# tangtang888/video-edge-ai-proxy

Measured on AMD Instinct MI355X. Metric: decoded FPS (whole node) + p50 VideoLatestImage latency, 256×1080p RTSP, higher is better.
Workload: dtype uint8 (BGR24 frames; bf16-capable consumer path)

## Files before the change

### csrc/bindings.cpp

```cpp
#include <malloc.h>

#include <pybind11/numpy.h>
#include <pybind11/pybind11.h>
#include <pybind11/stl.h>

#include "vep/hostprof.h"
#include "vep/avc.h"
#include "vep/avc_cavlc.h"
#include "vep/avc_recon.h"
#include "vep/bench_driver.h"
#include "vep/cabac.h"
#include "vep/codec.h"
#include "vep/gpu.h"
#include "vep/h264.h"
#include "vep/hevc_ctu.h"
#include "vep/hevc_dec.h"
#include "vep/hevc_kern.h"
#include "vep/jpeg.h"
#include "vep/scale.h"
#include "bind_ext.h"
#include "vep/runtime.h"
#include "vep/synth.h"

namespace py = pybind11;
// ... 837 lines not shown
  });
  m.def("parse_hevc_sps", [](const std::string& nal) {
    std::vector<u8> r(nal.size());
    size_t n = ebsp_to_rbsp(reinterpret_cast<const u8*>(nal.data()), nal.size(), r.data());
    hevc::Sps s = hevc::parse_sps(r.data(), n);
    py::dict d;
    d["profile_idc"] = s.ptl.profile_idc;
    d["level_idc"] = s.ptl.level_idc;
    d["width"] = s.out_width();
    d["height"] = s.out_height();
    d["coded_width"] = s.width;
    d["coded_height"] = s.height;
    d["fps"] = s.fps();
    d["ctb_size"] = s.ctb_size();
    d["pcm"] = s.pcm;
    d["num_short_term_rps"] = int(s.st_rps.size());
    d["scaling_list"] = s.scaling_list;
    d["scaling_list_data"] = s.scaling_list_data;
    d["long_term_refs"] = s.long_term_refs;
    d["num_long_term_ref_pics_sps"] = s.num_long_term_ref_pics_sps;
    return d;
  });
  auto hevc_rbsp = [](const std::string& nal) {
    std::vector<u8> r(nal.size());
    r.resize(ebsp_to_rbsp(reinterpret_cast<const u8*>(nal.data()), nal.size(), r.data()));
    return r;
  };
  m.def("parse_hevc_pps", [hevc_rbsp](const std::string& nal) {
    const std::vector<u8> r = hevc_rbsp(nal);
    hevc::Pps p = hevc::parse_pps(r.data(), r.size());
    py::dict d;
    d["tiles"] = p.tiles;
    d["tile_cols"] = p.tile_cols;
    d["tile_rows"] = p.tile_rows;
    d["uniform_spacing"] = p.uniform_spacing;
    d["loop_filter_across_tiles"] = p.loop_filter_across_tiles;
    d["entropy_coding_sync"] = p.entropy_coding_sync;
    d["dependent_slice_segments"] = p.dependent_slice_segments;
    d["weighted_pred"] = p.weighted_pred;
    d["weighted_bipred"] = p.weighted_bipred;
    d["transquant_bypass"] = p.transquant_bypass;
    d["scaling_list"] = p.scaling_list;
    return d;
  });
  m.def("hevc_scaling_factors", [hevc_rbsp](int size_id, int matrix_id, py::object sps_nal, py::object pps_nal) {
    VEP_CHECK(size_id >= 0 && size_id < 4 && matrix_id >= 0 && matrix_id < 6, "bad sizeId / matrixId");
    hevc::ScalingList sl;
    if (!sps_nal.is_none()) {
      const std::vector<u8> r = hevc_rbsp(sps_nal.cast<std::string>());
      sl = hevc::parse_sps(r.data(), r.size()).sl;
    }
    if (!pps_nal.is_none()) {
      const std::vector<u8> r = hevc_rbsp(pps_nal.cast<std::string>());
      hevc::Pps p = hevc::parse_pps(r.data(), r.size());
      if (p.scaling_list) sl = p.sl;
    }
    const int n = 4 << size_id;
    std::vector<u8> f(size_t(n) * n);
    sl.factors(size_id, matrix_id, f.data());
    return std::vector<int>(f.begin(), f.end());
  }, py::arg("size_id"), py::arg("matrix_id"), py::arg("sps_nal") = py::none(), py::arg("pps_nal") = py::none());
  m.def("hevc_slice_entry_points", [hevc_rbsp](const std::string& nal, const std::string& sps_nal,
                                               const std::string& pps_nal) {
    const std::vector<u8> rs = hevc_rbsp(sps_nal), rp = hevc_rbsp(pps_nal), r = hevc_rbsp(nal);
    const hevc::Sps sps = hevc::parse_sps(rs.data(), rs.size());
    const hevc::Pps pps = hevc::parse_pps(rp.data(), rp.size());
    const hevc::SliceHeader prev;
    const hevc::SliceHeader sh = hevc::parse_slice_header(r.data(), r.size(), sps, pps, &prev);
    size_t ebsp = 0, rbsp = 0;
    int zeros = 0;
    const u8* p = reinterpret_cast<const u8*>(nal.data());
    while (rbsp < sh.data_bytepos && ebsp < nal.size()) {
      const u8 b = p[ebsp++];
      if (zeros >= 2 && b == 3) {
        zeros = 0;
        continue;
      }
      ++rbsp;
      zeros = b == 0 ? zeros + 1 : 0;
    }
    py::dict d;
    d["entry_points"] = std::vector<u32>(sh.entry_points.begin(), sh.entry_points.end());
    d["data_offset_ebsp"] = ebsp;
    d["dependent"] = sh.dependent;
    d["segment_address"] = sh.segment_address;
    return d;
  });
  m.def("sparse_coef_fuzz", [](u64 seed, int trials) {
    u64 x = seed * 0x9E3779B97F4A7C15ull + 1;
    auto rnd = [&]() {
      x ^= x << 13;
      x ^= x >> 7;
      x ^= x << 17;
      return x;
    };
    auto val = [&](int density) -> i16 {
      if (int(rnd() & 15) >= density) return 0;
      const int r = int(rnd() % 8);
      if (r == 0) return i16(-32768);
      if (r == 1) return i16(32767);
      const int v = int(rnd() % 64) - 32;
      return i16(v ? v : 1);
    };
    int bad_avc = 0, bad_hevc = 0;
    for (int t = 0; t < trials; ++t) {
      const int dens = int(rnd() % 17);
      avc::MbResidual res;
      res.t8 = rnd() & 1;
      i16 want[avc::kDenseCoefs] = {};
      if (res.t8) {
        for (int q = 0; q < 4; ++q) {
          const bool coded = rnd() & 1;
          for (int i = 0; i < 64; ++i) want[64 * q + i] = res.b8[q][i] = coded ? val(dens) : 0;
          if (coded) res.luma |= u16(0x33u << ((q & 1) * 2 + (q >> 1) * 8));
        }
      } else {
        for (int b = 0; b < 16; ++b) {
          const bool coded = rnd() & 1;
          for (int i = 0; i < 16; ++i) want[16 * b + i] = res.blk[b][i] = coded ? val(dens) : 0;
          if (coded) res.luma |= u16(1u << b);
        }
      }
      for (int k = 0; k < 8; ++k) {
        const bool coded = rnd() & 1;
        for (int i = 0; i < 16; ++i) want[256 + 16 * k + i] = res.blk[16 + k][i] = coded ? val(dens) : 0;
        if (coded) res.chroma |= u8(1u << k);
      }
      avc::Picture pic;
      pic.wmbs = pic.hmbs = 1;
      pic.mbs.resize(1);
      avc::MbRec rec{};
      rec.kind = res.t8 ? avc::kI8x8 : avc::kI16x16;
      rec.flags = res.t8 ? u8(avc::kMbT8x8) : u8(0);
      avc::MbState s;
      avc::store_mb(pic, 0, rec, s, &res, nullptr);
      i16 got[avc::kDenseCoefs];
      avc::expand_coefs(pic.coefs.data(), pic.mbs[0], got);
      bad_avc += std::memcmp(got, want, sizeof got) != 0 ||
                 pic.coefs.size() != size_t(avc::coef_words(pic.mbs[0])) + avc::coef_values(pic.coefs.data(), pic.mbs[0]);
      for (int log2 = 2; log2 <= 5; ++log2) {
        const int nn = 1 << (2 * log2);
        std::vector<i16> dense(size_t(nn), 0), val_list, out(size_t(nn + nn / 16)), back(static_cast<size_t>(nn));
        std::vector<u16> pos;
        for (int k = 0; k < nn; ++k)
          if ((dense[size_t(k)] = val(dens))) pos.push_back(u16(k));
        for (size_t i = pos.size(); i > 1; --i) std::swap(pos[i - 1], pos[size_t(rnd() % i)]);
        for (u16 k : pos) val_list.push_back(dense[k]);
        const int n = hevc::hk_sparse_store(log2, pos.data(), val_list.data(), int(pos.size()), out.data());
        hevc::hk_sparse_expand(out.data(), log2, back.data());
        bad_hevc += back != dense || n != hevc::hk_sparse_words(log2) + int(pos.size());
      }
    }
    return std::make_pair(bad_avc, bad_hevc);
  });
  m.def("avc_parse_seconds", [](const std::vector<std::shared_ptr<AccessUnit>>& aus, int reps) {
    py::gil_scoped_release r;
    double best = 1e30;
    for (int k = 0; k < std::max(1, reps); ++k) {
      avc::Decoder dec;
      const i64 t0 = mono_us();
      for (const auto& au : aus) {
        size_t nal = 0;
        do dec.parse(*au, 0, &nal);
        while (nal < au->nals.size());
      }
      best = std::min(best, double(mono_us() - t0) * 1e-6);
    }
    return best;
  }, py::arg("aus"), py::arg("reps") = 3);
  m.def("avc_record_stats", [](const std::vector<std::shared_ptr<AccessUnit>>& aus) {
    py::gil_scoped_release r;
    avc::Decoder dec;
    u64 mbs = 0, coefs = 0, nz = 0, mvs = 0, pics = 0;
    for (const auto& au : aus) {
      auto p = dec.parse(*au);
      if (!p) continue;
      ++pics;
      mbs += p->mbs.size();
      coefs += p->coefs.size();
      mvs += p->mvs.size();
      for (const avc::MbRec& m : p->mbs)
        if (m.kind != avc::kIPcm) nz += avc::coef_values(p->coefs.data(), m);
    }
    py::gil_scoped_acquire g;
    py::dict d;
    d["pictures"] = pics;
    d["mbs"] = mbs;
    d["coefs"] = coefs;
    d["nonzero"] = nz;
    d["mvs"] = mvs;
    return d;
  });
  m.def("hevc_record_stats", [](const std::vector<std::shared_ptr<AccessUnit>>& aus) {
    py::gil_scoped_release r;
    hevc::Decoder dec;
    dec.set_gpu_mode(true);
    u64 pics = 0, tus = 0, coefs = 0, nz = 0, pus = 0;
    for (const auto& au : aus) {
      dec.decode(*au);
      for (const auto& p : dec.take_gpu_pictures()) {
        ++pics;
        tus += p->tus.size();
        pus += p->pus.size();
        coefs += p->coefs.size();
        for (i16 c : p->coefs) nz += c != 0;
      }
    }
    py::gil_scoped_acquire g;
    py::dict d;
    d["pictures"] = pics;
    d["tus"] = tus;
    d["coefs"] = coefs;
    d["nonzero"] = nz;
    d["pus"] = pus;
    return d;
  });
  m.def("avc_intra8x8_tap_check", [](u64 seed, int trials) {
    u64 st = seed * 0x9E3779B97F4A7C15ull + 7;
    auto rnd = [&]() {
      st ^= st << 13;
      st ^= st >> 7;
      st ^= st << 17;
      return int(st & 255);
    };
    int bad = 0;
    for (int t = 0; t < trials; ++t) {
      int s[25];
      for (int k = 0; k < 25; ++k) s[k] = (t & 3) == 0 ? (rnd() & 1) * 255 : rnd();
      auto T = [&](int i) { return s[1 + i]; };
      auto L = [&](int j) { return j < 0 ? s[0] : s[17 + j]; };
      for (int mode = 0; mode < 9; ++mode) {
        if (mode == 2) continue;
        for (int y = 0; y < 8; ++y)
          for (int x = 0; x < 8; ++x) {
            const u32 tw = avc::intra8x8_pred_tap(mode, x, y);
            const int got = avc::eval_tap8(tw, s[tw & 31], s[(tw >> 5) & 31], s[(tw >> 10) & 31]);
            bad += got != avc::intra8x8_pred_g(T, L, true, true, mode, x, y);
          }
      }
      for (int av = 0; av < 8; ++av) {
        const bool top = av & 1, left = av & 2, tl = av & 4;
        for (int k = 0; k < 25; ++k) {
          const u32 tw = avc::intra8x8_filter_tap(top, left, tl, k);
          const int got =
              (tw & avc::kTap8Const) ? 128 : avc::eval_tap8(tw, s[tw & 31], s[(tw >> 5) & 31], s[(tw >> 10) & 31]);
          bad += got != avc::intra8x8_filter_at(T, [&](int j) { return s[17 + j]; }, top, left, tl, k);
        }
      }
    }
    return bad;
  });
  m.def("cabac_roundtrip", [](u64 seed, int n, int qp) {
    u64 st = seed * 0x9E3779B97F4A7C15ull + 1;
    auto rnd = [&]() { st ^= st << 13; st ^= st >> 7; st ^= st << 17; return st; };
    const size_t nn = static_cast<size_t>(n);
    std::vector<u8> kind(nn), ctx(nn), bin(nn);
    for (int i = 0; i < n; ++i) {
      u64 r = rnd();
      kind[size_t(i)] = u8((r & 15) == 0 ? 1 : ((r & 63) == 1 ? 2 : 0));
      ctx[size_t(i)] = u8((r >> 8) % 4);
      const int p = ctx[size_t(i)] == 0 ? 2 : ctx[size_t(i)] == 1 ? 50 : ctx[size_t(i)] == 2 ? 97 : ((i / 500) & 1) ? 90 : 10;
      bin[size_t(i)] = kind[size_t(i)] == 2 ? 0 : u8(int((r >> 20) % 100) < p);
    }
    std::vector<u8> buf;
    cabac::Ctx ce[4], cd[4];
    const int init[4] = {197, 154, 122, 139};
    for (int k = 0; k < 4; ++k) ce[k].init(init[k], qp), cd[k].init(init[k], qp);
    {
      cabac::Encoder e(buf);
      for (int i = 0; i < n; ++i) {
        if (kind[size_t(i)] == 0) e.decision(ce[ctx[size_t(i)]], bin[size_t(i)]);
        else if (kind[size_t(i)] == 1) e.bypass(bin[size_t(i)]);
        else e.terminate(0);
      }
      e.terminate(1);
      e.align_zero();
    }
    cabac::Decoder d(buf.data(), buf.size(), 0);
    bool ok = true;
    for (int i = 0; i < n && ok; ++i) {
      u32 b;
      if (kind[size_t(i)] == 0) b = d.decision(cd[ctx[size_t(i)]]);
      else if (kind[size_t(i)] == 1) b = d.bypass();
      else b = d.terminate();
      ok = b == bin[size_t(i)];
    }
    ok = ok && d.terminate() == 1 && d.aligned_bytepos() == buf.size();
    return py::make_tuple(ok, buf.size());
  });
  m.def("parse_cost_us", [](const AccessUnit& au, int iters, std::shared_ptr<AccessUnit> prime) {
    py::gil_scoped_release r;
    StreamParser p;
    MbUpdate u;
    if (prime) p.absorb_parameter_sets(*prime);
    p.parse(au, u);
    i64 t0 = mono_us();
    for (int k = 0; k < iters; ++k) {
      u.clear_payload();
      p.parse(au, u);
    }
    const double parse_us = double(mono_us() - t0) / iters;
    std::vector<u32> epb;
    t0 = mono_us();
    for (int k = 0; k < iters; ++k)
      for (size_t i = 0; i < au.nals.size(); ++i) find_epb(au.nal(i), au.nal_size(i), epb);
    const double scan_us = double(mono_us() - t0) / iters;
// ... 1223 lines not shown
```

### csrc/vep/avc.cpp

```cpp
#include "avc.h"

#include <immintrin.h>

#include <algorithm>
#include <array>

#include "avc_cavlc.h"
#include "avc_internal.h"
#include "fanout.h"

namespace vep::avc {

using h264::Pps;
using h264::Sps;


void MbNeighbours::reset(int wmbs, int hmbs, bool ring) {
  w_ = wmbs;
  h_ = hmbs;
  cur_ = -1;
  run_slice_ = ~0u;
  run_start_ = 0;
  announced_ = 0;
  const size_t n = size_t(wmbs) * hmbs;
  if (++epoch_ == 0) {
    epoch_ = 1;
    stamp_.clear();
  }
  size_t ns = n;
  mask_ = ~size_t(0);
  if (ring) {
    size_t r = 1;
    while (r < 2 * (size_t(wmbs) + 2)) r <<= 1;
    if (r < n) {
      ns = r;
      mask_ = r - 1;
    }
  }
  if (st_.size() != ns) st_.assign(ns, MbState{});
  if (tag_.size() != ns) tag_.assign(ns, ~0u);
  if (stamp_.size() != n) stamp_.assign(n, 0u);
}

static int coded_count(const MbState& s, int blk) {
  if (s.kind == kSkip) return 0;
  if (s.kind == kIPcm) return 16;
  return s.tc[blk];
}

int MbNeighbours::nc_luma(int mb, int blk) const {
  const int bx = blk & 3, by = blk >> 2;
  int na = -1, nb = -1;
  const int am = mb_at(mb, bx * 4 - 1, by * 4);
  if (am >= 0) na = coded_count(st_[size_t(am) & mask_], bx > 0 ? blk - 1 : blk + 3);
  const int bm = mb_at(mb, bx * 4, by * 4 - 1);
  if (bm >= 0) nb = coded_count(st_[size_t(bm) & mask_], by > 0 ? blk - 4 : blk + 12);
  if (na >= 0 && nb >= 0) return (na + nb + 1) >> 1;
  if (na >= 0) return na;
  if (nb >= 0) return nb;
  return 0;
}

int MbNeighbours::nc_chroma(int mb, int c, int blk, int nbc) const {
  const int bx = blk & 1, by = blk >> 1;
  auto count = [&](int m, int b) {
    const MbState& s = st_[size_t(m) & mask_];
    if (s.kind == kSkip) return 0;
    if (s.kind == kIPcm) return 16;
    return int(s.tcc[c][b]);
  };
  int na = -1, nb = -1;
  const int am = bx > 0 ? mb : mb_at(mb, -1, 0);
  if (am >= 0) na = count(am, bx > 0 ? blk - 1 : blk + 1);
  const int bm = by > 0 ? mb : mb_at(mb, 0, -1);
  if (bm >= 0) nb = count(bm, by > 0 ? blk - 2 : blk + nbc - 2);
  if (na >= 0 && nb >= 0) return (na + nb + 1) >> 1;
  if (na >= 0) return na;
  if (nb >= 0) return nb;
  return 0;
}

int MbNeighbours::pred_intra4x4(int mb, int blk, bool constrained) const {
  const int bx = blk & 3, by = blk >> 2;
  const int am = mb_at(mb, bx * 4 - 1, by * 4), bm = mb_at(mb, bx * 4, by * 4 - 1);
  if (am < 0 || bm < 0) return 2;
  const MbState& a = st_[size_t(am) & mask_];
  const MbState& b = st_[size_t(bm) & mask_];
  if (constrained && (!is_intra(a.kind) || !is_intra(b.kind))) return 2;
  const int ma = a.kind == kI4x4 ? a.i4[bx > 0 ? blk - 1 : blk + 3] : 2;
  const int mbm = b.kind == kI4x4 ? b.i4[by > 0 ? blk - 4 : blk + 12] : 2;
  return ma < mbm ? ma : mbm;
}

int MbNeighbours::pred_intra8x8(int mb, int b8, bool constrained) const {
  const int blk = (b8 & 1) * 2 + (b8 >> 1) * 8;
  const int bx = blk & 3, by = blk >> 2;
  const int am = mb_at(mb, bx * 4 - 1, by * 4), bm = mb_at(mb, bx * 4, by * 4 - 1);
  if (am < 0 || bm < 0) return 2;
  const MbState& a = st_[size_t(am) & mask_];
  const MbState& b = st_[size_t(bm) & mask_];
  if (constrained && (!is_intra(a.kind) || !is_intra(b.kind))) return 2;
  auto mode = [](const MbState& n, int r, int b8n) -> int {
    if (n.kind == kI8x8) return n.i4[(b8n & 1) * 2 + (b8n >> 1) * 8];
    if (n.kind == kI4x4) return n.i4[r];
    return 2;
  };
  const int ra = bx > 0 ? blk - 1 : blk + 3, rb = by > 0 ? blk - 4 : blk + 12;
  const int b8a = ((ra >> 3) << 1) | ((ra & 3) >> 1), b8b = ((rb >> 3) << 1) | ((rb & 3) >> 1);
  const int ma = mode(a, ra, b8a), mbm = mode(b, rb, b8b);
  return ma < mbm ? ma : mbm;
}

static int median3(int a, int b, int c) { return a + b + c - std::min({a, b, c}) - std::max({a, b, c}); }

void MbNeighbours::pred_mv(int mb, int x4, int y4, int w4, int h4, int list, int ref, u16 done, int shape,
                           int out[2]) const {
  (void)h4;
  if (mb == cur_ && w4 == 4 && h4 == 4 && shape == 0) return pred_mv16(list, ref, out);
  const int x = x4 * 4, y = y4 * 4, w = w4 * 4;
  Nb A = motion_at(mb, x - 1, y, done, list);
  Nb B = motion_at(mb, x, y - 1, done, list);
  Nb C = motion_at(mb, x + w, y - 1, done, list);
  if (!C.avail) C = motion_at(mb, x - 1, y - 1, done, list);
  auto take = [&](const Nb& n) {
    out[0] = n.mv[0];
    out[1] = n.mv[1];
  };
  if (shape == 1) {
    if (y4 == 0 && B.ref == ref) return take(B);
    if (y4 != 0 && A.ref == ref) return take(A);
  } else if (shape == 2) {
    if (x4 == 0 && A.ref == ref) return take(A);
    if (x4 != 0 && C.ref == ref) return take(C);
  }
  if (!B.avail && !C.avail && A.avail) B = C = A;
  const int match = (A.ref == ref) + (B.ref == ref) + (C.ref == ref);
  if (match == 1) return take(A.ref == ref ? A : B.ref == ref ? B : C);
  out[0] = median3(A.mv[0], B.mv[0], C.mv[0]);
  out[1] = median3(A.mv[1], B.mv[1], C.mv[1]);
}

void MbNeighbours::pskip_mv(int mb, int out[2]) const {
  out[0] = out[1] = 0;
  if (mb == cur_) {
    if (a_ < 0 || b_ < 0) return;
    Nb n[3];
    nb16(0, n);
    if ((n[0].ref == 0 && n[0].mv[0] == 0 && n[0].mv[1] == 0) || (n[1].ref == 0 && n[1].mv[0] == 0 && n[1].mv[1] == 0))
      return;
    pred_mv16(0, 0, out);
    return;
  }
  if (mb_at(mb, -1, 0) < 0 || mb_at(mb, 0, -1) < 0) return;
  const Nb A = motion_at(mb, -1, 0, 0, 0), B = motion_at(mb, 0, -1, 0, 0);
  if ((A.ref == 0 && A.mv[0] == 0 && A.mv[1] == 0) || (B.ref == 0 && B.mv[0] == 0 && B.mv[1] == 0))
    return;
  pred_mv(mb, 0, 0, 4, 4, 0, 0, 0, 0, out);
}
// ... 831 lines not shown
      const int dqp = br.se();
      VEP_CHECK(dqp >= -26 && dqp <= 25, "mb_qp_delta out of range");
      qp = (qp + dqp + 52) % 52;
      qp_out_ = qp;
    }
    s.qp = u8(qp);
    residual(br, mb, s, res, cbp_luma, cbp_chroma, qp);
    emit(mb, s, res, i16_mode, chroma_mode);
  }

  int qp_out_ = -1;

 private:
  int read_ref(Bits& br) {
    const int n = sc_.sh.num_ref_idx[0];
    int r = 0;
    if (n == 2) r = int(br.u1() ^ 1u);
    else if (n > 2) r = int(br.ue());
    VEP_CHECK(r < n && sc_.list0[size_t(r)].slot >= 0, "ref_idx_l0 names a missing reference picture");
    return r;
  }

  void set_part(MbState& s, int x4, int y4, int w4, int h4, const int mv[2]) {
    for (int y = y4; y < y4 + h4; ++y)
      for (int x = x4; x < x4 + w4; ++x) {
        s.mv[0][y * 4 + x][0] = i16(mv[0]);
        s.mv[0][y * 4 + x][1] = i16(mv[1]);
      }
  }
  static u16 part_mask(int x4, int y4, int w4, int h4) {
    u16 m = 0;
    for (int y = y4; y < y4 + h4; ++y)
      for (int x = x4; x < x4 + w4; ++x) m |= u16(1u << (y * 4 + x));
    return m;
  }

  void inter_pred(Bits& br, int mb, MbState& s, int mbt) {
    struct Part {
      int x4, y4, w4, h4, ref, shape;
      int mvd[2];
    };
    Part parts[16];
    int np = 0;
    if (mbt <= 2) {
      const int n = mbt == 0 ? 1 : 2;
      int refs[2] = {0, 0};
      for (int i = 0; i < n; ++i) refs[i] = read_ref(br);
      for (int i = 0; i < n; ++i) {
        Part& p = parts[np++];
        p.ref = refs[i];
        p.mvd[0] = br.se();
        p.mvd[1] = br.se();
        if (mbt == 0) p.x4 = 0, p.y4 = 0, p.w4 = 4, p.h4 = 4, p.shape = 0;
        else if (mbt == 1) p.x4 = 0, p.y4 = 2 * i, p.w4 = 4, p.h4 = 2, p.shape = 1;
        else p.x4 = 2 * i, p.y4 = 0, p.w4 = 2, p.h4 = 4, p.shape = 2;
      }
      for (int i = 0; i < n; ++i) {
        const Part& p = parts[i];
        for (int y = p.y4 / 2; y < (p.y4 + p.h4) / 2; ++y)
          for (int x = p.x4 / 2; x < (p.x4 + p.w4) / 2; ++x) s.ref[0][y * 2 + x] = i8(p.ref);
      }
    } else {
      int sub[4], refs[4];
      for (int& t : sub) {
        t = int(br.ue());
        VEP_CHECK(t <= 3, "bad P sub_mb_type");
      }
      for (int i = 0; i < 4; ++i) refs[i] = mbt == 4 ? 0 : read_ref(br);
      for (int i = 0; i < 4; ++i) {
        s.ref[0][i] = i8(refs[i]);
        const int x8 = (i & 1) * 2, y8 = (i >> 1) * 2;
        const int cnt = sub[i] == 0 ? 1 : sub[i] == 3 ? 4 : 2;
        for (int j = 0; j < cnt; ++j) {
          Part& p = parts[np++];
          p.ref = refs[i];
          p.shape = 0;
          p.mvd[0] = br.se();
          p.mvd[1] = br.se();
          switch (sub[i]) {
            case 0: p.x4 = x8, p.y4 = y8, p.w4 = 2, p.h4 = 2; break;
            case 1: p.x4 = x8, p.y4 = y8 + j, p.w4 = 2, p.h4 = 1; break;
            case 2: p.x4 = x8 + j, p.y4 = y8, p.w4 = 1, p.h4 = 2; break;
            default: p.x4 = x8 + (j & 1), p.y4 = y8 + (j >> 1), p.w4 = 1, p.h4 = 1; break;
          }
        }
      }
    }
    u16 done = 0;
    for (int i = 0; i < np; ++i) {
      const Part& p = parts[i];
      int mvp[2];
      nb_.pred_mv(mb, p.x4, p.y4, p.w4, p.h4, 0, p.ref, done, p.shape, mvp);
      int mv[2] = {mvp[0] + p.mvd[0], mvp[1] + p.mvd[1]};
      VEP_CHECK(mv[0] >= -32768 && mv[0] <= 32767 && mv[1] >= -32768 && mv[1] <= 32767,
                "motion vector out of range");
      set_part(s, p.x4, p.y4, p.w4, p.h4, mv);
      done |= part_mask(p.x4, p.y4, p.w4, p.h4);
    }
  }

  static constexpr u8 kNa = 0xFF;
  u8 ncl_[25];
  u8 ncc_[2][9];

  void nc_setup(int mb) {
    std::memset(ncl_, 0, sizeof ncl_);
    std::memset(ncc_, 0, sizeof ncc_);
    const int am = nb_.mb_at(mb, -1, 0), bm = nb_.mb_at(mb, 0, -1);
    const MbState* a = am >= 0 ? &nb_.at(am) : nullptr;
    const MbState* b = bm >= 0 ? &nb_.at(bm) : nullptr;
    for (int k = 0; k < 4; ++k) {
      ncl_[1 + k] = b ? b->tc[12 + k] : kNa;
      ncl_[(k + 1) * 5] = a ? a->tc[k * 4 + 3] : kNa;
    }
    ncl_[0] = kNa;
    for (int c = 0; c < 2; ++c) {
      for (int k = 0; k < 2; ++k) {
        ncc_[c][1 + k] = b ? b->tcc[c][2 + k] : kNa;
        ncc_[c][(k + 1) * 3] = a ? a->tcc[c][k * 2 + 1] : kNa;
      }
      ncc_[c][0] = kNa;
    }
  }
  static int nc_of(u8 na, u8 nb) {
    if (na != kNa && nb != kNa) return (na + nb + 1) >> 1;
    if (na != kNa) return na;
    if (nb != kNa) return nb;
    return 0;
  }
  int ncl(int r) const {
    const int i = ((r >> 2) + 1) * 5 + (r & 3) + 1;
    return nc_of(ncl_[i - 1], ncl_[i - 5]);
  }
  int ncc(int c, int b) const {
    const int i = ((b >> 1) + 1) * 3 + (b & 1) + 1;
    return nc_of(ncc_[c][i - 1], ncc_[c][i - 3]);
  }

  struct Scale {
    const int* ls;
    int mul, add, sh;
  };

  void residual(Bits& br, int mb, MbState& s, MbResidual& res, int cbp_luma, int cbp_chroma, int qp) {
    res.luma = 0;
    res.chroma = 0;
    nc_setup(mb);
    const bool intra16 = s.kind == kI16x16;
    auto scaler = [](int q) {
      return Scale{kLevelScale[q % 6], q >= 24 ? 1 << (q / 6 - 4) : 1, q >= 24 ? 0 : 1 << (3 - q / 6),
                   q >= 24 ? 0 : 4 - q / 6};
    };
    const auto dl = scaler(qp);
    auto luma_block = [&](int r, int start, int max_coeff, int dcv) {
      i16* d = res.blk[r];
      std::memset(d, 0, 16 * sizeof(i16));
      bool nz = dcv != 0;
      d[0] = sat16(dcv);
      const int tc = read_residual_block_cb(br, ncl(r), max_coeff, [&](int k, int l) {
        const int pos = kZigzag4x4[k + start];
        const int v = (l * dl.ls[pos] * dl.mul + dl.add) >> dl.sh;
        d[pos] = sat16(v);
        nz |= v != 0;
      });
      s.tc[r] = u8(tc);
      ncl_[((r >> 2) + 1) * 5 + (r & 3) + 1] = u8(tc);
      if (nz) res.luma |= u16(1u << r);
    };
    if (intra16) {
      int c[16] = {};
      const bool have_dc =
          read_residual_block_cb(br, ncl(0), 16, [&](int k, int l) { c[kZigzag4x4[k]] = l; }) > 0;
      int dcy[16] = {};
      if (have_dc) {
        hadamard4x4(c);
        const int ls = 16 * kNormAdjust[qp % 6][0];
        for (int k = 0; k < 16; ++k)
          dcy[k] = qp >= 36 ? c[k] * ls * (1 << (qp / 6 - 6)) : (c[k] * ls + (1 << (5 - qp / 6))) >> (6 - qp / 6);
      }
      for (int idx = 0; idx < 16; ++idx) {
        const int r = blk_to_raster(idx);
        if (cbp_luma) {
          luma_block(r, 1, 15, dcy[r]);
        } else if (dcy[r] != 0) {
          i16* d = res.blk[r];
          std::memset(d, 0, 16 * sizeof(i16));
          d[0] = sat16(dcy[r]);
          res.luma |= u16(1u << r);
        }
      }
    } else {
      for (int idx = 0; idx < 16; ++idx)
        if ((cbp_luma >> (idx >> 2)) & 1) luma_block(blk_to_raster(idx), 0, 16, 0);
    }
    if (cbp_chroma) {
      const int qpc = chroma_qp(qp, sc_.pps.chroma_qp_index_offset);
      const auto dc = scaler(qpc);
      const int ls = 16 * kNormAdjust[qpc % 6][0];
      int dcv[2][4];
      for (int c = 0; c < 2; ++c) {
        int v[4] = {0, 0, 0, 0};
        read_residual_block_cb(br, -1, 4, [&](int k, int l) { v[k] = l; });
        const int f[4] = {v[0] + v[1] + v[2] + v[3], v[0] - v[1] + v[2] - v[3],
                          v[0] + v[1] - v[2] - v[3], v[0] - v[1] - v[2] + v[3]};
        for (int b = 0; b < 4; ++b) dcv[c][b] = ((f[b] * ls) * (1 << (qpc / 6))) >> 5;
      }
      for (int c = 0; c < 2; ++c)
        for (int b = 0; b < 4; ++b) {
          i16* d = res.blk[16 + c * 4 + b];
          bool nz = dcv[c][b] != 0;
          if (cbp_chroma & 2) {
            std::memset(d, 0, 16 * sizeof(i16));
            d[0] = sat16(dcv[c][b]);
            const int tc = read_residual_block_cb(br, ncc(c, b), 15, [&](int k, int l) {
              const int pos = kZigzag4x4[k + 1];
              const int v = (l * dc.ls[pos] * dc.mul + dc.add) >> dc.sh;
              d[pos] = sat16(v);
              nz |= v != 0;
            });
            s.tcc[c][b] = u8(tc);
            ncc_[c][((b >> 1) + 1) * 3 + (b & 1) + 1] = u8(tc);
          } else if (nz) {
            std::memset(d, 0, 16 * sizeof(i16));
            d[0] = sat16(dcv[c][b]);
          }
          if (nz) res.chroma |= u8(1u << (c * 4 + b));
        }
    }
    VEP_CHECK(!br.overrun(), "slice data overrun");
  }

  void emit(int mb, const MbState& s, const MbResidual& res, int i16_mode, int chroma_mode) {
    MbRec m{};
    m.kind = s.kind;
    m.qp = s.kind == kIPcm ? 0 : s.qp;
    m.qpc = u8(chroma_qp(m.qp, sc_.pps.chroma_qp_index_offset));
    m.qpc2 = m.qpc;
    m.i16_mode = u8(i16_mode);
    m.chroma_mode = u8(chroma_mode);
    m.dbk = u8((sc_.sh.disable_deblocking == 1 ? 1 : 0) | (sc_.sh.disable_deblocking == 2 ? 2 : 0));
    m.alpha_off = i8(sc_.sh.alpha_off);
    m.beta_off = i8(sc_.sh.beta_off);
    m.slice = s.slice;
    for (int k = 0; k < 4; ++k) {
      m.ref[k] = s.ref[0][k] >= 0 ? u8(sc_.list0[size_t(s.ref[0][k])].slot) : u8(0xFF);
      m.ref1[k] = u8(0xFF);
    }
    for (int r = 0; r < 16; ++r) m.i4[r >> 1] |= u8((s.kind == kI4x4 ? s.i4[r] : 0) << ((r & 1) * 4));
    for (int r = 0; r < 16; ++r) m.nz |= u16(s.tc[r] ? 1u << r : 0u);
    store_mb(pic_, mb, m, s, &res, pcm_, nullptr);
  }

  MbNeighbours& nb_;
  Picture& pic_;
  const SliceCtx& sc_;
  const u8* pcm_ = nullptr;
};

}

namespace {

bool legacy_slice(const SliceHdr& sh, const Sps& sps, const Pps& pps) {
  return !pps.cabac && !sh.field_pic && sps.chroma_format_idc == 1 && sps.bit_depth_luma == 8 && (sh.type() == h264::kP || sh.type() == h264::kI) && !pps.transform_8x8_mode &&
         !sps.scaling_matrix_present && !pps.scaling_matrix_present && !sh.explicit_wp &&
         pps.chroma_qp_index_offset == pps.second_chroma_qp_index_offset;
}

int dpb_slots_for(const Sps& sps) {
  int bound;
  if (sps.max_num_reorder_frames >= 0) bound = sps.max_num_reorder_frames;
  else if (sps.poc_type == 2 || sps.profile_idc == 66) bound = 0;
  else bound = sps.max_dpb_frames();
  return std::min(kMaxDpbSlots, std::max(1, sps.max_num_ref_frames) + bound + 2);
}

}

static void validate_picture(const Picture& p);

struct Decoder::SliceUnit {
  MbNeighbours nb;
  Picture shard;
  ColBuild colb;
  std::vector<u8> rbsp;
  SliceHdr sh;
  const Sps* sps = nullptr;
  const Pps* pps = nullptr;
  size_t bitpos = 0;
  int slice_idx = 0;
  std::vector<ListEntry> list[2];
  std::array<std::vector<u32>, 2> uids;
};

PicturePtr Decoder::parse(const AccessUnit& au, i64 tag, size_t* next_nal) {
  struct FenceOnExit {
    ~FenceOnExit() {
#if defined(__x86_64__)
      _mm_sfence();
#endif
    }
  } fence;
  auto pic = pic_pool_->acquire([](Picture& p) {
    auto mbs = std::move(p.mbs);
    auto coefs = std::move(p.coefs), mvs = std::move(p.mvs);
    auto wps = std::move(p.wps);
    std::vector<OutFrame> outputs = std::move(p.outputs);
    p = Picture{};
    coefs.clear();
    mvs.clear();
    wps.clear();
    outputs.clear();
    p.mbs = std::move(mbs);
    p.coefs = std::move(coefs);
    p.mvs = std::move(mvs);
    p.wps = std::move(wps);
    p.outputs = std::move(outputs);
  });
  bool got = false;
  bool hard_flush = false;
  bool second_field = false;
  int slice_idx = 0;
  SliceHdr first;
  const Sps* act_sps = nullptr;
  const Pps* act_pps = nullptr;
  std::vector<u8> scratch;
  std::vector<std::array<std::vector<u32>, 2>> slice_uids;
  ColBuild colb;
  std::shared_ptr<ColMotion> col_built;
  struct ColbGuard {
    Picture* p;
    ~ColbGuard() { p->colb = nullptr; }
  } colb_guard{pic.get()};
  int nslices = 0;
  for (size_t i = 0; i < au.nals.size(); ++i)
    if (au.nal_size(i) >= 2) {
      const int t = h264::nal_type(au.nal(i)[0]);
      nslices += (t == h264::kNalSlice || t == h264::kNalIdr) ? 1 : 0;
    }
  const bool par = parallel_slices_ && nslices >= 2 && FanOut::shared().size() > 0;
  int nunits = 0;
  const size_t start = next_nal ? *next_nal : 0;
  if (next_nal) *next_nal = au.nals.size();
  for (size_t i = start; i < au.nals.size(); ++i) {
    const u8* p = au.nal(i);
    const size_t n = au.nal_size(i);
    if (n < 2) continue;
    const int t = h264::nal_type(p[0]);
    if (t == h264::kNalSps || t == h264::kNalPps) {
      size_t rn;
      const u8* r = unescape(p, n, epb_, scratch, rn);
      if (t == h264::kNalSps) {
        Sps s = h264::parse_sps(r, rn);
        check_sps_supported(s);
        sps_[s.sps_id] = s;
      } else {
        Pps q = h264::parse_pps(r, rn);
        pps_[q.pps_id] = q;
      }
      continue;
    }
    if (t >= 2 && t <= 4) throw UnsupportedStream("H.264 data partitioning is not supported");
    if (t != h264::kNalSlice && t != h264::kNalIdr) continue;
    size_t rn;
    const u32 *kb = nullptr, *ke = nullptr;
    au.epb_of(i, &kb, &ke);
    const u8* r = unescape(p, n, epb_, rbsp_, rn, kb, ke);
    Bits peek(r + 1, rn - 1);
    peek.ue();
    peek.ue();
    const int pps_id = int(peek.ue());
    auto pit = pps_.find(pps_id);
    if (pit == pps_.end()) throw UnsupportedStream("slice references unknown PPS");
    auto sit = sps_.find(pit->second.sps_id);
    if (sit == sps_.end()) throw UnsupportedStream("slice references unknown SPS");
    const Sps& sps = sit->second;
    const Pps& pps = pit->second;
    check_sps_supported(sps);
    Bits br(r + 1, rn - 1);
    const SliceHdr sh = read_slice_header(br, p[0], sps, pps);
    if (sh.redundant_pic_cnt > 0) {
      ++redundant_slices_skipped;
// ... 170 lines not shown
    });
    parallel_slices_run_ += u64(nunits);
    covered.assign(size_t(pic->nmbs()), 0);
    for (int k = 0; k < nunits; ++k) {
      SliceUnit& u = *units_[size_t(k)];
      const Picture& sh = u.shard;
      const u32 coef0 = u32(pic->coefs.size()), mv0 = u32(pic->mvs.size()), wp0 = u32(pic->wps.size());
      const u32 res0 = u32(pic->intra_res);
      pic->coefs.insert(pic->coefs.end(), sh.coefs.begin(), sh.coefs.end());
      pic->mvs.insert(pic->mvs.end(), sh.mvs.begin(), sh.mvs.end());
      pic->wps.insert(pic->wps.end(), sh.wps.begin(), sh.wps.end());
      pic->intra_mbs += sh.intra_mbs;
      pic->intra_res += sh.intra_res;
      pic->inter_mbs += sh.inter_mbs;
      pic->deblock |= sh.deblock;
      for (int mb = u.sh.first_mb; mb < pic->nmbs(); ++mb) {
        if (!u.nb.announced(mb)) continue;
        VEP_CHECK(!covered[size_t(mb)], "H.264: slices overlap");
        covered[size_t(mb)] = 1;
        MbRec m = sh.mbs[size_t(mb)];
        m.coef += coef0;
        if (m.kind == kSkip || m.kind == kInter) m.mv += mv0;
        if (m.flags & kMbWp) m.wp += wp0;
        if (m.res != kNoRes) m.res += res0;
        pic->mbs[size_t(mb)] = m;
      }
    }
  }
  int ncovered = 0;
  if (par)
    for (u8 c : covered) ncovered += c;
  auto announced = [&](int mb) { return par ? covered[size_t(mb)] != 0 : nb_.announced(mb); };
  int missing = 0;
  for (int mb = 0; (par ? ncovered : nb_.announced_count()) < pic->nmbs() && mb < pic->nmbs(); ++mb) {
    MbRec& m = pic->mbs[size_t(mb)];
    if (announced(mb)) continue;
    ++missing;
    if (pic->colb) colb.none(mb);
    m = MbRec{};
    m.res = kNoRes;
    m.dbk = 1;
    m.slice = u16(0xFFFF);
    std::fill(std::begin(m.ref1), std::end(m.ref1), u8(0xFF));
    if (!dpb_.empty()) {
      m.kind = kSkip;
      int cs = dpb_.front().slot;
      if (pic->structure) {
        const int par = pic->structure - 1;
        cs = 2 * cs + ((((dpb_.front().fields | dpb_.front().lt_fields) >> par) & 1) ? par : 1 - par);
      }
      for (auto& rf : m.ref) rf = u8(cs);
      m.mv = u32(pic->mvs.size());
      m.flags |= kMbMv16;
      pic->mvs.resize(pic->mvs.size() + 2, 0);
      ++pic->inter_mbs;
    } else {
      m.kind = kI16x16;
      m.i16_mode = 2;
      std::fill(std::begin(m.ref), std::end(m.ref), u8(0xFF));
      ++pic->intra_mbs;
    }
  }
  pic->info.coded_mbs = pic->nmbs() - missing;
  const u32 uid = next_uid_++;
  if (first.field_pic) {
    if (first.nal_ref_idc != 0)
      mark_field(first, *act_sps, pic->target >> 1, pic->poc, uid, second_field && pair_.ref, std::move(col_built));
    if (first.has_mmco5() && !second_field) {
      pic->poc = 0;
      pair_.frame_num = 0;
      pair_.poc[int(first.bottom_field)] = 0;
      pair_.boundary = true;
      pair_.hard = reorder_cur_ == 0;
    }
    if (second_field) close_pair(*pic);
  } else {
    if (first.nal_ref_idc != 0) {
      mark_references(first, *act_sps, pic->target, pic->poc, uid, std::move(col_built));
    }
    const bool boundary = first.idr() || first.has_mmco5();
    if (first.has_mmco5()) pic->poc = 0;
    bump(*pic, out_of(*pic), boundary, boundary && (hard_flush || reorder_cur_ == 0));
  }
  if (missing || par) validate(*pic);
  else validate_picture(*pic);
  return pic;
}

Decoder::Decoder() {
  if (const char* e = std::getenv("VEP_AVC_SLICE_THREADS")) parallel_slices_ = e[0] != '0';
}
Decoder::~Decoder() = default;

void Decoder::parse_slice_data(MbNeighbours& nb, Picture& pic, const SliceHdr& sh, const Sps& sps, const Pps& pps,
                               const u8* data, size_t n, size_t bitpos, int slice_idx,
                               const std::vector<ListEntry> (&lists)[2]) {
  if (legacy_slice(sh, sps, pps)) {
    Bits br(data, n, bitpos);
    const size_t stop = BitReader(data, n).stop_bit_pos();
    SliceCtx sc{sh, pps, slice_idx, sh.type() == h264::kP, sh.qp, lists[0]};
    const int total = pic.nmbs();
    int mb = sh.first_mb;
    VEP_CHECK(mb < total, "first_mb_in_slice past end of picture");
    bool more = true;
    while (more) {
      if (sc.is_p) {
        const u32 run = br.ue();
        VEP_CHECK(u32(total - mb) >= run, "mb_skip_run past end of picture");
        MbDecoder d(nb, pic, sc);
        for (u32 k = 0; k < run; ++k) d.skip(mb++);
        if (run > 0) {
          more = br.pos() < stop;
          if (!more) break;
        }
      }
      VEP_CHECK(mb < total, "macroblock address past end of picture");
      MbDecoder d(nb, pic, sc);
      d.macroblock(br, mb);
      if (d.qp_out_ >= 0) sc.qp = d.qp_out_;
      VEP_CHECK(!br.overrun(), "slice data overrun");
      more = br.pos() < stop;
      ++mb;
    }
    return;
  }
  SliceEnv env;
  env.sh = &sh;
  env.sps = &sps;
  env.pps = &pps;
  env.slice = slice_idx;
  env.list[0] = &lists[0];
  env.list[1] = &lists[1];
  env.cur_poc = pic.poc;
  env.scaling = h264::resolve_scaling(sps, pps);
  env.field = sh.field_pic;
  decode_slice_generic(nb, pic, env, data, n, bitpos);
}

static inline void validate_mb(const Picture& p, const MbRec& m, bool written = false) {
  const size_t ncoef = p.coefs.size(), nmv = p.mvs.size();
  VEP_CHECK(m.kind <= kI8x8, "macroblock kind out of range");
  VEP_CHECK(p.cf == 2 || m.chroma_coded < 0x100, "chroma block mask out of range");
  VEP_CHECK(m.qp <= 51 + p.qp_bias && m.qpc <= 51 + p.qpc_bias && m.qpc2 <= 51 + p.qpc_bias,
            "macroblock QP out of range");
  if (m.kind == kIPcm) {
    const size_t ns = p.cf == 2 ? size_t(kPcmMaxSamples) : size_t(kPcmMbBytes);
    VEP_CHECK(size_t(m.coef) + (p.bd > 8 ? ns : ns / 2) <= ncoef, "I_PCM samples outside the pool");
    return;
  }
  const size_t nw = size_t(coef_words(m));
  VEP_CHECK(size_t(m.coef) + nw <= ncoef, "coefficient masks outside the pool");
  VEP_CHECK(written || size_t(m.coef) + nw + coef_values(p.coefs.data(), m) <= ncoef, "coefficients outside the pool");
  VEP_CHECK(m.chroma_mode <= 3 && m.i16_mode <= 3, "intra prediction mode out of range");
  if (m.flags & kMbT8x8)
    for (int q = 0; q < 4; ++q) {
      const u32 g = (u32(m.luma_coded) >> ((q & 1) * 2 + (q >> 1) * 8)) & 0x33u;
      VEP_CHECK(g == 0 || g == 0x33u, "8x8 residual block partially coded");
    }
  if (m.kind == kSkip || m.kind == kInter) {
    VEP_CHECK(size_t(m.mv) + size_t(mv_per_list(m.flags)) * ((m.flags & kMbL1) ? 2 : 1) <= nmv,
              "motion vectors outside the pool");
    for (int k = 0; k < 4; ++k) {
      const int r0 = m.ref[k], r1 = m.ref1[k];
      VEP_CHECK(r0 != 0xFF || r1 != 0xFF, "inter partition without a reference");
      VEP_CHECK((r0 == 0xFF || r0 < p.dpb_slots) && (r1 == 0xFF || r1 < p.dpb_slots),
                "reference slot outside the DPB");
      VEP_CHECK(r1 == 0xFF || (m.flags & kMbL1), "list-1 reference without list-1 motion");
    }
    if (m.flags & kMbWp) VEP_CHECK(size_t(m.wp) + 4 <= p.wps.size(), "weights outside the pool");
  } else if (m.kind == kI4x4) {
    for (u8 b : m.i4) VEP_CHECK((b & 15) <= 8 && (b >> 4) <= 8, "Intra_4x4 mode out of range");
  } else if (m.kind == kI8x8) {
    VEP_CHECK((m.flags & kMbT8x8) && (m.i4[0] & 15) <= 8 && (m.i4[0] >> 4) <= 8 && (m.i4[1] & 15) <= 8 &&
                  (m.i4[1] >> 4) <= 8,
              "Intra_8x8 mode out of range");
  }
  VEP_CHECK(m.res == kNoRes || (is_intra(m.kind) && m.res < u32(p.intra_res)), "residual slot out of range");
}

static inline void validate_written_mb(const Picture& p, const MbRec& m) {
  const size_t ncoef = p.coefs.size(), nmv = p.mvs.size();
  bool ok = (m.kind <= kI8x8) & (p.cf == 2 || m.chroma_coded < 0x100) & (m.qp <= 51 + p.qp_bias) &
            (m.qpc <= 51 + p.qpc_bias) & (m.qpc2 <= 51 + p.qpc_bias);
  if (m.kind != kIPcm) {
    ok &= size_t(m.coef) + size_t(coef_words(m)) <= ncoef;
    ok &= (m.chroma_mode <= 3) & (m.i16_mode <= 3);
    if (m.flags & kMbT8x8)
      for (int q = 0; q < 4; ++q) {
        const u32 g = (u32(m.luma_coded) >> ((q & 1) * 2 + (q >> 1) * 8)) & 0x33u;
        ok &= (g == 0) | (g == 0x33u);
      }
    if (m.kind == kSkip || m.kind == kInter) {
      ok &= size_t(m.mv) + size_t(mv_per_list(m.flags)) * ((m.flags & kMbL1) ? 2 : 1) <= nmv;
      u32 r0w, r1w;
      std::memcpy(&r0w, m.ref, 4);
      std::memcpy(&r1w, m.ref1, 4);
      for (int k = 0; k < 4; ++k) {
        const u32 r0 = (r0w >> (8 * k)) & 0xFFu, r1 = (r1w >> (8 * k)) & 0xFFu;
        ok &= (r0 != 0xFF) | (r1 != 0xFF);
        ok &= (r0 == 0xFF) | (r0 < u32(p.dpb_slots));
        ok &= (r1 == 0xFF) | (r1 < u32(p.dpb_slots));
        ok &= (r1 == 0xFF) | ((m.flags & kMbL1) != 0);
      }
      if (m.flags & kMbWp) ok &= size_t(m.wp) + 4 <= p.wps.size();
    } else if (m.kind == kI4x4 || m.kind == kI8x8) {
      for (u8 b : m.i4) ok &= ((b & 15) <= 8) & ((b >> 4) <= 8);
      if (m.kind == kI8x8) ok &= (m.flags & kMbT8x8) != 0;
    }
    ok &= m.res == kNoRes || (is_intra(m.kind) && m.res < u32(p.intra_res));
  }
  if (!ok) validate_mb(p, m, true);
}

static void validate_picture(const Picture& p) {
  VEP_CHECK(p.dpb_slots >= 1 && p.dpb_slots <= kMaxDpbSlots && p.target >= 0 && p.target < p.dpb_slots,
            "picture DPB slots out of range");
  VEP_CHECK(p.wmbs > 0 && p.hmbs > 0 && p.mbs.size() == size_t(p.nmbs()), "picture size mismatch");
}

void validate(const Picture& p) {
  validate_picture(p);
  for (const MbRec& m : p.mbs) validate_mb(p, m);
}


static inline void stream_words(void* dst, const void* src, size_t bytes) {
#if defined(__x86_64__)
  long long w[16];
  for (size_t o = 0; o < bytes; o += sizeof w) {
    const size_t n = bytes - o < sizeof w ? bytes - o : sizeof w;
    std::memcpy(w, static_cast<const char*>(src) + o, n);
    long long* d = reinterpret_cast<long long*>(static_cast<char*>(dst) + o);
    for (size_t k = 0; k < n / 8; ++k) _mm_stream_si64(d + k, w[k]);
  }
#else
  std::memcpy(dst, src, bytes);
#endif
}

void ColBuild::none(int mb) {
  const int per = col->corners ? 4 : 16;
  ColMotion::Blk* out = &col->b[size_t(mb) * size_t(per)];
  for (int k = 0; k < per; ++k) out[k] = ColMotion::Blk{{0, 0}, 0u, i8(-1)};
}

void ColBuild::store(int mb, const MbState& st) {
  if (is_intra(st.kind) || !uids) {
    none(mb);
    return;
  }
  static constexpr u8 kCorner[4] = {0, 3, 12, 15};
  const auto& lu = *uids;
  if (col->corners) {
    ColMotion::Blk out[4];
    for (int k = 0; k < 4; ++k) {
      const int l = st.ref[0][k] >= 0 ? 0 : 1;
      const int ri = st.ref[l][k];
      out[k] = ri < 0 ? ColMotion::Blk{{0, 0}, 0u, i8(-1)}
                      : ColMotion::Blk{{st.mv[l][kCorner[k]][0], st.mv[l][kCorner[k]][1]}, uid_tab[l][ri & 31], i8(ri)};
    }
    stream_words(&col->b[size_t(mb) * 4], out, sizeof out);
    return;
  }
  ColMotion::Blk* out = &col->b[size_t(mb) * 16];
  for (int blk = 0; blk < 16; ++blk) {
    const int b8 = ((blk >> 3) << 1) | ((blk & 3) >> 1);
    const int l = st.ref[0][b8] >= 0 ? 0 : 1;
    const int ri = st.ref[l][b8];
    if (ri < 0) {
      out[blk] = ColMotion::Blk{{0, 0}, 0u, i8(-1)};
      continue;
    }
    out[blk] = ColMotion::Blk{{st.mv[l][blk][0], st.mv[l][blk][1]},
                              size_t(ri) < lu[size_t(l)].size() ? lu[size_t(l)][size_t(ri)] : 0u, i8(ri)};
  }
}

std::shared_ptr<ColMotion> build_col_motion(const MbNeighbours& nb, int wmbs, int hmbs,
                                            const std::vector<std::array<std::vector<u32>, 2>>& slice_uids,
                                            bool corners, Recycler<ColMotion>* pool) {
  auto col = pool ? pool->acquire([](ColMotion&) {}) : std::make_shared<ColMotion>();
  col->wmbs = wmbs;
  col->hmbs = hmbs;
  col->corners = corners;
  const int per = corners ? 4 : 16;
  col->b.resize(size_t(wmbs) * hmbs * size_t(per));
  static constexpr u8 kCorner[4] = {0, 3, 12, 15};
  for (int mb = 0; mb < wmbs * hmbs; ++mb) {
    const MbState& st = nb.at(mb);
    ColMotion::Blk* out = &col->b[size_t(mb) * size_t(per)];
    if (!nb.decoded(mb) || is_intra(st.kind) || slice_uids.empty()) {
      for (int k = 0; k < per; ++k) out[k] = ColMotion::Blk{{0, 0}, 0u, i8(-1)};
      continue;
    }
    const auto& lu = slice_uids[std::min<size_t>(st.slice, slice_uids.size() - 1)];
    for (int k = 0; k < per; ++k) {
      const int blk = corners ? kCorner[k] : k;
      const int b8 = ((blk >> 3) << 1) | ((blk & 3) >> 1);
      const int l = st.ref[0][b8] >= 0 ? 0 : 1;
      const int ri = st.ref[l][b8];
      if (ri < 0) {
        out[k] = ColMotion::Blk{{0, 0}, 0u, i8(-1)};
        continue;
      }
      out[k] = ColMotion::Blk{{st.mv[l][blk][0], st.mv[l][blk][1]},
                              size_t(ri) < lu[size_t(l)].size() ? lu[size_t(l)][size_t(ri)] : 0u, i8(ri)};
    }
  }
  return col;
}

namespace {
template <class P>
const P* yplane(const HostSurface& s) {
  if constexpr (sizeof(P) == 1) return s.y.data();
  else return s.y16.data();
}
template <class P>
const P* uvplane(const HostSurface& s) {
  if constexpr (sizeof(P) == 1) return s.uv.data();
  else return s.uv16.data();
}
template <class P>
P* yplane(HostSurface& s) {
  if constexpr (sizeof(P) == 1) return s.y.data();
  else return s.y16.data();
}
template <class P>
P* uvplane(HostSurface& s) {
  if constexpr (sizeof(P) == 1) return s.uv.data();
  else return s.uv16.data();
}

template <class P>
void predict_inter_t(const std::vector<HostSurface>& slots, const MbRec& m, const i16* mv0, const i16* mv1,
                     const WpEntry* wp, int mx, int my, int* py, int (*pc)[128], int structure, int bd) {
  auto cy_off = [&](int slot) { return structure ? 2 * ((structure == 2) - (slot & 1)) : 0; };
  const int pitch = slots[0].coded_w, wpx = pitch, hpx = slots[0].coded_h;
  for (int y = 0; y < 16; ++y)
// ... 55 lines not shown
    const int dcv = have_dc ? dcy[r] : 0;
    if (!ac && dcv == 0) continue;
    i16* d = res.blk[r];
    std::memset(d, 0, 16 * sizeof(i16));
    bool nz = dcv != 0;
    d[0] = sat16(dcv);
    if (ac) {
      for (int k = i16x16 ? 1 : 0; k < 16; ++k) {
        const int l = lv.luma[r][k];
        if (!l) continue;
        const int pos = kZigzag4x4[k];
        const int v = dequant4x4(l, qp, pos >> 2, pos & 3);
        d[pos] = sat16(v);
        nz |= v != 0;
      }
    }
    if (nz) res.luma |= u16(1u << r);
  }
  (void)q6;
  (void)qm;
  const int ls = 16 * kNormAdjust[qpc % 6][0];
  for (int c = 0; c < 2; ++c) {
    const bool has_dc = (lv.dcmask >> (1 + c)) & 1;
    const int acm = (lv.cmask >> (c * 4)) & 15;
    if (!has_dc && !acm) continue;
    int f[4] = {0, 0, 0, 0};
    if (has_dc) {
      const int c0 = lv.cdc[c][0], c1 = lv.cdc[c][1], c2 = lv.cdc[c][2], c3 = lv.cdc[c][3];
      f[0] = c0 + c1 + c2 + c3;
      f[1] = c0 - c1 + c2 - c3;
      f[2] = c0 + c1 - c2 - c3;
      f[3] = c0 - c1 - c2 + c3;
    }
    for (int b = 0; b < 4; ++b) {
      const int dcv = ((f[b] * ls) * (1 << (qpc / 6))) >> 5;
      const bool ac = (acm >> b) & 1;
      if (!ac && dcv == 0) continue;
      i16* d = res.blk[16 + c * 4 + b];
      std::memset(d, 0, 16 * sizeof(i16));
      d[0] = sat16(dcv);
      bool nz = dcv != 0;
      if (ac) {
        for (int k = 1; k < 16; ++k) {
          const int l = lv.cac[c][b][k];
          if (!l) continue;
          const int pos = kZigzag4x4[k];
          const int v = dequant4x4(l, qpc, pos >> 2, pos & 3);
          d[pos] = sat16(v);
          nz |= v != 0;
        }
      }
      if (nz) res.chroma |= u8(1u << (c * 4 + b));
    }
  }
}

static inline u16 nonzero_mask16(const i16* p) {
#if defined(__AVX2__) && defined(__BMI2__)
  const __m256i v = _mm256_loadu_si256(reinterpret_cast<const __m256i*>(p));
  const u32 zero = u32(_mm256_movemask_epi8(_mm256_cmpeq_epi16(v, _mm256_setzero_si256())));
  return u16(_pext_u32(~zero, 0x55555555u));
#else
  u32 m = 0;
  for (int i = 0; i < 16; ++i) m |= u32(p[i] != 0) << i;
  return u16(m);
#endif
}

struct Compact8 {
  alignas(16) u8 c[256][16];
  constexpr Compact8() : c() {
    for (int m = 0; m < 256; ++m) {
      int k = 0;
      for (int i = 0; i < 8; ++i)
        if ((m >> i) & 1) {
          c[m][2 * k] = u8(2 * i);
          c[m][2 * k + 1] = u8(2 * i + 1);
          ++k;
        }
      for (int j = 2 * k; j < 16; ++j) c[m][j] = 0x80;
    }
  }
};
static constexpr Compact8 kCompact8{};

static inline i16* compact16(const i16* p, u32 mask, i16* out) {
#if defined(__SSSE3__)
  const __m128i lo = _mm_loadu_si128(reinterpret_cast<const __m128i*>(p));
  const __m128i hi = _mm_loadu_si128(reinterpret_cast<const __m128i*>(p + 8));
  const u32 m0 = mask & 0xFFu, m1 = mask >> 8;
  _mm_storeu_si128(reinterpret_cast<__m128i*>(out),
                   _mm_shuffle_epi8(lo, _mm_load_si128(reinterpret_cast<const __m128i*>(kCompact8.c[m0]))));
  out += __builtin_popcount(m0);
  _mm_storeu_si128(reinterpret_cast<__m128i*>(out),
                   _mm_shuffle_epi8(hi, _mm_load_si128(reinterpret_cast<const __m128i*>(kCompact8.c[m1]))));
  return out + __builtin_popcount(m1);
#else
  for (int i = 0; i < 16; ++i) {
    *out = p[i];
    out += (mask >> i) & 1;
  }
  return out;
#endif
}

static inline u32 motion_uniformity(const i16* mv) {
#if defined(__AVX2__)
  const __m256i a = _mm256_loadu_si256(reinterpret_cast<const __m256i*>(mv));
  const __m256i b = _mm256_loadu_si256(reinterpret_cast<const __m256i*>(mv + 16));
  const __m256i v0 = _mm256_broadcastd_epi32(_mm256_castsi256_si128(a));
  const __m256i tl = _mm256_setr_epi32(0, 0, 2, 2, 0, 0, 2, 2);
  const u32 all = u32(_mm256_movemask_epi8(_mm256_and_si256(_mm256_cmpeq_epi32(a, v0), _mm256_cmpeq_epi32(b, v0))));
  const u32 q8 = u32(_mm256_movemask_epi8(_mm256_and_si256(_mm256_cmpeq_epi32(a, _mm256_permutevar8x32_epi32(a, tl)),
                                                           _mm256_cmpeq_epi32(b, _mm256_permutevar8x32_epi32(b, tl)))));
  return (all == 0xFFFFFFFFu ? 1u : 0u) | (q8 == 0xFFFFFFFFu ? 2u : 0u);
#else
  u32 v[16];
  std::memcpy(v, mv, sizeof v);
  bool u16 = true, u8x8 = true;
  for (int b = 1; b < 16; ++b) u16 &= v[b] == v[0];
  for (int b = 0; b < 16; ++b) u8x8 &= v[b] == v[((b >> 3) << 3) | (b & 2)];
  return (u16 ? 1u : 0u) | (u8x8 ? 2u : 0u);
#endif
}

static inline void store_motion(Picture& pic, MbRec& m, const MbState& s) {
  const int nl = (m.flags & kMbL1) ? 2 : 1;
  u32 u = 3;
  for (int l = 0; l < nl; ++l) u &= motion_uniformity(&s.mv[l][0][0]);
  m.flags |= (u & 1) ? kMbMv16 : ((u & 2) ? kMbMv8x8 : 0);
  m.mv = u32(pic.mvs.size());
  const int per = (u & 1) ? 2 : ((u & 2) ? 8 : 32);
  i16* out = pic.mvs.extend(size_t(per * nl));
  for (int l = 0; l < nl; ++l, out += per) {
    const i16* v = &s.mv[l][0][0];
    if (per == 2) {
      std::memcpy(out, v, 4);
    } else if (per == 8) {
      std::memcpy(out, v, 4);
      std::memcpy(out + 2, v + 4, 4);
      std::memcpy(out + 4, v + 16, 4);
      std::memcpy(out + 6, v + 20, 4);
    } else {
      std::memcpy(out, v, 64);
    }
  }
}

static inline void store_rec(MbRec* dst, const MbRec& m) {
  static_assert(sizeof(MbRec) % 8 == 0 && sizeof(ColMotion::Blk) * 4 % 8 == 0, "8-byte words");
  stream_words(dst, &m, sizeof(MbRec));
}

void store_skip_mb(Picture& pic, int mb, MbRec& m, const MbState& s) {
  m.coef = u32(pic.coefs.size());
  m.luma_coded = 0;
  m.chroma_coded = 0;
  m.wp = 0;
  m.res = kNoRes;
  store_motion(pic, m, s);
  ++pic.inter_mbs;
  if (!(m.dbk & 1)) pic.deblock = true;
  for (int k = 0; k < 4; ++k) {
    const int r0 = m.ref[k], r1 = m.ref1[k];
    VEP_CHECK((r0 != 0xFF || r1 != 0xFF) && (r0 == 0xFF || r0 < pic.dpb_slots) && (r1 == 0xFF || r1 < pic.dpb_slots) &&
                  (r1 == 0xFF || (m.flags & kMbL1)),
              "skipped macroblock reference slot outside the DPB");
  }
  VEP_CHECK(m.qp <= 51 + pic.qp_bias && m.qpc <= 51 + pic.qpc_bias && m.qpc2 <= 51 + pic.qpc_bias,
            "macroblock QP out of range");
  store_rec(&pic.mbs[size_t(mb)], m);
  if (pic.colb) pic.colb->store(mb, s);
}

void store_mb(Picture& pic, int mb, MbRec m, const MbState& s, const MbResidual* res, const u8* pcm,
              const WpEntry* wp) {
  m.coef = u32(pic.coefs.size());
  m.luma_coded = 0;
  m.chroma_coded = 0;
  if (m.kind == kIPcm) {
    VEP_CHECK(pcm, "I_PCM macroblock without samples");
    const size_t ns = pic.cf == 2 ? size_t(kPcmMaxSamples) : size_t(kPcmMbBytes);
    const size_t o = pic.coefs.size(), nb = pic.bd > 8 ? 2 * ns : ns;
    pic.coefs.resize(o + nb / 2);
    std::memcpy(pic.coefs.data() + o, pcm, nb);
  } else if (res && (res->luma | res->chroma)) {
    m.luma_coded = res->luma;
    m.chroma_coded = res->chroma;
    if (res->t8) m.flags |= kMbT8x8;
    const i16* grp[32];
    int ng = 0;
    if (res->t8) {
      for (int q = 0; q < 4; ++q)
        if ((res->luma >> ((q & 1) * 2 + (q >> 1) * 8)) & 1)
          for (int w = 0; w < 4; ++w) grp[ng++] = res->b8[q] + 16 * w;
    } else {
      for (u32 w = res->luma; w; w &= w - 1) grp[ng++] = res->blk[__builtin_ctz(w)];
    }
    for (u32 w = res->chroma; w; w &= w - 1) grp[ng++] = res->blk[16 + __builtin_ctz(w)];
    u16 mask[32];
    int nv = 0;
    for (int g = 0; g < ng; ++g) {
      mask[g] = nonzero_mask16(grp[g]);
      nv += __builtin_popcount(mask[g]);
    }
    const size_t o = pic.coefs.size();
    i16* out = pic.coefs.extend(size_t(ng + nv) + 8);
    std::memcpy(out, mask, size_t(ng) * sizeof(u16));
    i16* v = out + ng;
    for (int g = 0; g < ng; ++g) v = compact16(grp[g], mask[g], v);
    pic.coefs.resize(o + size_t(ng + nv));
  }
  m.mv = 0;
  m.wp = 0;
  m.flags &= u8(~(kMbMv8x8 | kMbMv16));
  if (m.kind == kSkip || m.kind == kInter) {
    store_motion(pic, m, s);
    if (wp && (m.flags & kMbWp)) {
      m.wp = u32(pic.wps.size());
      pic.wps.insert(pic.wps.end(), wp, wp + 4);
    } else {
      m.flags &= u8(~kMbWp);
    }
    ++pic.inter_mbs;
  } else if (m.kind == kIPcm) {
    ++pic.inter_mbs;
  } else {
    ++pic.intra_mbs;
  }
  m.res = is_intra(m.kind) && m.kind != kIPcm && (m.luma_coded | m.chroma_coded) ? u32(pic.intra_res++) : kNoRes;
  if (!(m.dbk & 1)) pic.deblock = true;
  validate_written_mb(pic, m);
  store_rec(&pic.mbs[size_t(mb)], m);
  if (pic.colb) pic.colb->store(mb, s);
}


namespace {

bool intra_avail(const Picture& pic, const MbRec& m, int nx, int ny) {
  if (nx < 0 || ny < 0 || nx >= pic.wmbs) return false;
  const MbRec& n = pic.mbs[size_t(ny) * pic.wmbs + nx];
  if (n.slice != m.slice) return false;
  return !(pic.constrained_intra && !is_intra(n.kind));
}

const i16* luma_res(const i16* dense, const MbRec& m, int r) {
  if (!((m.luma_coded >> r) & 1)) return nullptr;
  return dense + 16 * r;
}

const i16* chroma_res(const i16* dense, const MbRec& m, int c, int b, int nbc) {
  const int k = c * nbc + b;
  if (!((m.chroma_coded >> k) & 1)) return nullptr;
  return dense + 256 + 16 * k;
}

void luma_residual(const i16* dense, const MbRec& m, int* out) {
  std::memset(out, 0, 256 * sizeof(int));
  if (m.flags & kMbT8x8) {
    for (int q = 0; q < 4; ++q) {
      if (!((m.luma_coded >> ((q & 1) * 2 + (q >> 1) * 8)) & 1)) continue;
      int r[64];
      idct8x8(dense + 64 * q, r);
      for (int i = 0; i < 8; ++i)
        for (int j = 0; j < 8; ++j) out[((q >> 1) * 8 + i) * 16 + (q & 1) * 8 + j] = r[i * 8 + j];
    }
    return;
  }
  for (int blk = 0; blk < 16; ++blk) {
    const i16* d = luma_res(dense, m, blk);
    if (!d) continue;
    int r[16];
    idct4x4(d, r);
    for (int i = 0; i < 4; ++i)
      for (int j = 0; j < 4; ++j) out[((blk >> 2) * 4 + i) * 16 + (blk & 3) * 4 + j] = r[i * 4 + j];
  }
}

template <class P>
struct Recon {
  const Picture& pic;
  std::vector<HostSurface>& slots;
  HostSurface& T;
  int pitch, wpx, hpx, bd;
  int cf, ch, nbc;
  i16 dense[kDenseCoefs];

  void load(const MbRec& m) {
    if (m.kind != kIPcm) expand_coefs(pic.coefs.data(), m, dense);
  }

  P& Y(int x, int y) { return yplane<P>(T)[size_t(y) * pitch + x]; }
  P& C(int x, int y, int c) { return uvplane<P>(T)[size_t(y) * pitch + 2 * x + c]; }
  P px(int v) const { return P(clip1(v, bd)); }

  void chroma_store(const MbRec& m, int mx, int my, int c, const int* pred ) {
    for (int b = 0; b < nbc; ++b) {
      const i16* d = chroma_res(dense, m, c, b, nbc);
      int res[16] = {};
      if (d) idct4x4(d, res);
      const int bx = (b & 1) * 4, by = (b >> 1) * 4;
      for (int i = 0; i < 4; ++i)
        for (int j = 0; j < 4; ++j)
          C(mx * 8 + bx + j, my * ch + by + i, c) = px(pred[(by + i) * 8 + bx + j] + res[i * 4 + j]);
    }
  }

  void inter(const MbRec& m, int mx, int my) {
    i16 e[2][32];
    const i16* base = &pic.mvs[size_t(m.mv)];
    for (int l = 0; l < ((m.flags & kMbL1) ? 2 : 1); ++l)
      for (int b = 0; b < 16; ++b) {
        const i16* v = base + mv_sub(m.flags, l, b);
        e[l][2 * b] = v[0];
        e[l][2 * b + 1] = v[1];
      }
    const i16* mv0 = e[0];
    const i16* mv1 = (m.flags & kMbL1) ? e[1] : nullptr;
    const WpEntry* wp = (m.flags & kMbWp) ? &pic.wps[m.wp] : nullptr;
    int py[256], pc[2][128], res[256];
    predict_inter_t<P>(slots, m, mv0, mv1, wp, mx, my, py, pc, pic.structure, bd);
    luma_residual(dense, m, res);
    for (int y = 0; y < 16; ++y)
      for (int x = 0; x < 16; ++x) Y(mx * 16 + x, my * 16 + y) = px(py[y * 16 + x] + res[y * 16 + x]);
    for (int c = 0; c < 2; ++c) chroma_store(m, mx, my, c, pc[c]);
  }

  void pcm(const MbRec& m, int mx, int my) {
    const P* s = reinterpret_cast<const P*>(pic.coefs.data() + m.coef);
    for (int y = 0; y < 16; ++y)
      for (int x = 0; x < 16; ++x) Y(mx * 16 + x, my * 16 + y) = s[y * 16 + x];
    for (int c = 0; c < 2; ++c)
      for (int y = 0; y < ch; ++y)
        for (int x = 0; x < 8; ++x) C(mx * 8 + x, my * ch + y, c) = s[256 + c * 8 * ch + y * 8 + x];
  }

  void intra_chroma(const MbRec& m, int mb, int mx, int my) {
// ... 250 lines not shown
```

### csrc/vep/avc.h

```cpp
#pragma once

#include <array>
#include <map>
#include <memory>

#include "hostmem.h"
#include "recycle.h"
#include "avc_recon.h"
#include "codec.h"

namespace vep::avc {

constexpr int kMaxDpbSlots = 34;

struct AuMeta {
  i64 pts = 0, dts = 0, arrival_ms = 0;
  i64 tag = 0;
  bool keyframe = false, corrupt = false;
};

struct OutFrame {
  int slot = -1;
  PictureInfo info;
  AuMeta au;
// ... 325 lines not shown
  }
};

struct ColBuild {
  ColMotion* col = nullptr;
  const std::array<std::vector<u32>, 2>* uids = nullptr;
  u32 uid_tab[2][32] = {};
  void set_uids(const std::array<std::vector<u32>, 2>* u) {
    uids = u;
    for (int l = 0; l < 2; ++l)
      for (size_t k = 0; k < 32; ++k) uid_tab[l][k] = u && k < (*u)[size_t(l)].size() ? (*u)[size_t(l)][k] : 0u;
  }
  void store(int mb, const MbState& st);
  void none(int mb);
};

struct RefPic {
  int slot = -1;
  int frame_num = 0;
  int frame_num_wrap = 0;
  bool long_term = false;
  int lt_idx = 0;
  int poc = 0;
  u32 uid = 0;
  std::shared_ptr<const ColMotion> col;
  u8 fields = 3;
  u8 lt_fields = 0;
  int poc_f[2] = {0, 0};
  u32 uid_f[2] = {0, 0};
  std::shared_ptr<const ColMotion> col_f[2];
};

struct ListEntry {
  int slot = -1;
  int poc = 0;
  bool long_term = false;
  u32 uid = 0;
  const ColMotion* col = nullptr;
};

class Decoder {
 public:
  PicturePtr parse(const AccessUnit& au, i64 tag = 0, size_t* next_nal = nullptr);
  void absorb_parameter_sets(const AccessUnit& au);
  bool has_sps() const { return !sps_.empty(); }
  void reset_references();
  int dpb_slots() const { return dpb_slots_; }
  int pending_output() const { return int(pending_.size()); }
  std::vector<OutFrame> flush_output();

 private:
  struct Pending {
    OutFrame f;
    u32 epoch;
  };
  void build_lists(const SliceHdr& sh, const h264::Sps& sps, int cur_poc);
  void build_field_lists(const SliceHdr& sh, const h264::Sps& sps, int cur_poc);
  void mark_field(const SliceHdr& sh, const h264::Sps& sps, int slot, int poc, u32 uid, bool second,
                  std::shared_ptr<const ColMotion> col);
  void mark_references(const SliceHdr& sh, const h264::Sps& sps, int slot, int poc, u32 uid,
                       std::shared_ptr<const ColMotion> col);
  int pick_slot() const;
  int compute_poc(const SliceHdr& sh, const h264::Sps& sps);
  void bump(Picture& pic, const OutFrame& f, bool new_epoch, bool hard);
  OutFrame out_of(const Picture& pic) const;
  int reorder_depth(const h264::Sps& sps) const;
  void parse_slice_data(MbNeighbours& nb, Picture& pic, const SliceHdr& sh, const h264::Sps& sps,
                        const h264::Pps& pps, const u8* data, size_t n, size_t bitpos, int slice_idx,
                        const std::vector<ListEntry> (&lists)[2]);

  std::map<int, h264::Sps> sps_;
  std::map<int, h264::Pps> pps_;
  std::vector<u8> rbsp_;
  std::vector<u32> epb_;
  MbNeighbours nb_;
  std::vector<RefPic> dpb_;
  std::shared_ptr<Recycler<Picture>> pic_pool_ = Recycler<Picture>::make(12);
  std::shared_ptr<Recycler<ColMotion>> col_pool_ = Recycler<ColMotion>::make(8);
  std::vector<Pending> pending_;
  std::vector<ListEntry> list_[2];
  int max_lt_idx_ = -1;
  int dpb_slots_ = 2;
  int wmbs_ = 0, hmbs_ = 0;
  int bd_ = 8;
  int cf_ = 1;
  bool have_idr_ = false;
  int pinned_slot_ = -1;
  int last_out_poc_ = 0;
  i64 last_out_epoch_ = -1;
  u32 epoch_ = 0;
  int adaptive_reorder_ = 0;
  int reorder_cur_ = 0;
  u32 next_uid_ = 1;
  int prev_poc_msb_ = 0, prev_poc_lsb_ = 0;
  int prev_frame_num_ = 0, prev_frame_num_offset_ = 0;
  bool prev_ref_mmco5_ = false;
  std::vector<std::vector<MbState>> spare_;
  struct SliceUnit;
  bool parallel_slices_ = true;
  std::vector<std::unique_ptr<SliceUnit>> units_;
  u64 parallel_slices_run_ = 0;
  bool field_mode_ = false;
  struct OpenPair {
    bool open = false;
    int slot = -1, frame_num = 0, bottom = 0;
    int poc[2] = {0, 0};
    bool ref = false, boundary = false, hard = false;
    u8 have = 0;
    OutFrame f;
  } pair_;
  void close_pair(Picture& pic);

 public:
  Decoder();
  ~Decoder();
  u64 parallel_slices_run() const { return parallel_slices_run_; }
  u64 mmco_ops[7] = {0, 0, 0, 0, 0, 0, 0};
  u64 list_mods = 0, long_term_marked = 0;
  u64 redundant_slices_skipped = 0;
};

void cpu_reconstruct(const Picture& pic, std::vector<HostSurface>& slots);
void weave_fields(const HostSurface& top, const HostSurface& bottom, HostSurface& frame);

struct MbLevels {
  int luma[16][16];
  int dc[16];
  int cdc[2][4];
  int cac[2][4][16];
  u16 lmask = 0;
  u8 cmask = 0;
  u8 dcmask = 0;
  void update_masks() {
    lmask = cmask = dcmask = 0;
    for (int r = 0; r < 16; ++r)
      for (int k = 0; k < 16; ++k)
        if (luma[r][k]) lmask |= u16(1u << r);
    for (int k = 0; k < 16; ++k)
      if (dc[k]) dcmask |= 1;
    for (int c = 0; c < 2; ++c)
      for (int b = 0; b < 4; ++b) {
        if (cdc[c][b]) dcmask |= u8(2 << c);
        for (int k = 0; k < 16; ++k)
          if (cac[c][b][k]) cmask |= u8(1u << (c * 4 + b));
      }
  }
};
struct MbResidual {
  i16 blk[32][16];
  i16 b8[4][64];
  u16 luma = 0;
  u16 chroma = 0;
  bool t8 = false;
};
void dequantize_mb(const MbLevels& lv, bool i16x16, int qp, int qpc, MbResidual& out);
void store_mb(Picture& pic, int mb, MbRec m, const MbState& s, const MbResidual* res, const u8* pcm,
              const WpEntry* wp = nullptr);
void store_skip_mb(Picture& pic, int mb, MbRec& m, const MbState& s);
void cpu_reconstruct_mb(const Picture& pic, int mb, std::vector<HostSurface>& slots);
void cpu_deblock(const Picture& pic, HostSurface& target);
void intra4x4_neighbours(const Picture& pic, int mb, int idx, const HostSurface& T, Intra4Nb& n);
void intra16_neighbours(const Picture& pic, int mb, const HostSurface& T, Intra16Nb& n);
void chroma_neighbours(const Picture& pic, int mb, int c, const HostSurface& T, IntraChromaNb& n);
void intra8x8_neighbours(const Picture& pic, int mb, int q, const HostSurface& T, int* f, bool& has_top,
                         bool& has_left);

class StreamEncoder {
 public:
  virtual ~StreamEncoder() = default;
  virtual std::shared_ptr<AccessUnit> next() = 0;
  virtual const HostSurface& reconstruction() const = 0;
  virtual const HostSurface& source() const = 0;
  virtual i64 last_pts() const = 0;
  virtual const std::vector<u8>& sps_nal() const = 0;
  virtual const std::vector<u8>& pps_nal() const = 0;
};

struct AvcEncConfig {
  int width = 640, height = 480;
  int fps = 30, gop = 30;
  int idr_phase = 0;
  int qp = 28;
  int slices = 1;
  int refs = 1;
  int objects = 3;
  u64 seed = 1;
  int deblock_idc = 0;
  int alpha_off = 0, beta_off = 0;
  bool constrained_intra = false;
  int chroma_qp_offset = 0;
  bool coverage = false;
  int pcm_rate = 0;
  int nonref_rate = 0;
  double noise = 3.0;
  double temporal_noise = 0;
};

class AvcEncoder : public StreamEncoder {
 public:
  explicit AvcEncoder(const AvcEncConfig& cfg);
  ~AvcEncoder() override;
  std::shared_ptr<AccessUnit> next() override;
  const HostSurface& reconstruction() const override;
  const HostSurface& source() const override;
  i64 last_pts() const override;
  const AvcEncConfig& config() const { return cfg_; }
  const std::vector<u8>& sps_nal() const override;
  const std::vector<u8>& pps_nal() const override;

 private:
  struct Impl;
  AvcEncConfig cfg_;
  std::unique_ptr<Impl> p_;
};

struct AvcHighConfig {
  int width = 640, height = 480;
  int fps = 30, gop = 30;
  int idr_phase = 0;
  int bframes = 2;
  bool pyramid = true;
  int refs = 2;
  int qp = 28;
  bool cabac = true;
  bool t8x8 = true;
  bool weighted_p = false;
  int weighted_b = 0;
  bool direct_spatial = true;
  bool scaling = false;
  int slices = 1;
  int deblock_idc = 0;
  int chroma_qp_offset = 0, second_chroma_qp_offset = 0;
  bool coverage = false;
  bool interlaced = false;
  bool marking = false;
  bool fields = false;
  bool mono = false;
  int bit_depth = 8;
  int chroma_format = 1;
  int objects = 3;
  double noise = 3.0, temporal_noise = 0.0;
  u64 seed = 1;
};

class AvcHighEncoder : public StreamEncoder {
 public:
  explicit AvcHighEncoder(const AvcHighConfig& cfg);
  ~AvcHighEncoder() override;
  std::shared_ptr<AccessUnit> next() override;
  const HostSurface& reconstruction() const override;
  const HostSurface& source() const override;
  i64 last_pts() const override;
  i64 last_display_index() const;
  char last_type() const;
  const AvcHighConfig& config() const { return cfg_; }
  const std::vector<u8>& sps_nal() const override;
  const std::vector<u8>& pps_nal() const override;

 private:
  struct Impl;
  AvcHighConfig cfg_;
  std::unique_ptr<Impl> p_;
};

}
```

### csrc/vep/avc_internal.h

```cpp
#pragma once

#include <array>

#include "avc.h"
#include "bits.h"

namespace vep::avc {

struct SliceEnv {
  const SliceHdr* sh = nullptr;
  const h264::Sps* sps = nullptr;
  const h264::Pps* pps = nullptr;
  int slice = 0;
  const std::vector<ListEntry>* list[2] = {nullptr, nullptr};
  int cur_poc = 0;
  h264::ScalingLists scaling;
  bool field = false;
};

void decode_slice_generic(MbNeighbours& nb, Picture& pic, const SliceEnv& env, const u8* data, size_t n,
                          size_t bitpos);

WpEntry wp_entry(const SliceEnv& env, int r0, int r1);

std::shared_ptr<ColMotion> build_col_motion(const MbNeighbours& nb, int wmbs, int hmbs,
                                            const std::vector<std::array<std::vector<u32>, 2>>& slice_uids,
                                            bool corners, Recycler<ColMotion>* pool = nullptr);

void predict_inter(const std::vector<HostSurface>& slots, const MbRec& m, const i16* mv0, const i16* mv1,
                   const WpEntry* wp, int mx, int my, int* py, int (*pc)[128], int structure = 0);

struct MbDesc {
  bool skip = false;
  int mb_type = 0;
  int sub[4] = {0, 0, 0, 0};
  bool t8x8 = false;
  u8 ipred[16] = {};
  int chroma_mode = 0;
  int ref[2][4] = {{0, 0, 0, 0}, {0, 0, 0, 0}};
  i16 mv[2][16][2] = {};
  int cbp = 0;
  int qp_delta = 0;
  int dc[16] = {};
  int ac[16][16] = {};
  int l8[4][64] = {};
  int cdc[2][8] = {};
  int cac[2][8][15] = {};
  const u8* pcm = nullptr;
};

class SliceWriter {
 public:
  SliceWriter(MbNeighbours& nb, Picture& pic, const SliceEnv& env, BitWriter& bw);
  ~SliceWriter();
  void write_mb(int mb, const MbDesc& d);
  void finish();
  void skip_motion(int mb, MbState& out);
  int qp() const;

 private:
  struct Impl;
  std::unique_ptr<Impl> p_;
};

inline i16 sat16(int v) { return i16(v < -32768 ? -32768 : v > 32767 ? 32767 : v); }

inline void hadamard4x4(int c[16]) {
  int t[16];
  for (int i = 0; i < 4; ++i) {
    const int a = c[i * 4], b = c[i * 4 + 1], d = c[i * 4 + 2], e = c[i * 4 + 3];
    t[i * 4] = a + b + d + e;
    t[i * 4 + 1] = a + b - d - e;
    t[i * 4 + 2] = a - b - d + e;
    t[i * 4 + 3] = a - b + d - e;
  }
  for (int j = 0; j < 4; ++j) {
    const int a = t[j], b = t[4 + j], d = t[8 + j], e = t[12 + j];
    c[j] = a + b + d + e;
    c[4 + j] = a + b - d - e;
    c[8 + j] = a - b - d + e;
    c[12 + j] = a - b + d - e;
  }
}

}
```

### csrc/vep/avc_mb.cpp

```cpp
#include <algorithm>
#include <memory>
#include <cstddef>
#include <cstring>

#include "avc_cabac.h"
#include "avc_cavlc.h"
#include "avc_internal.h"

namespace vep::avc {

namespace {

struct Dequant {
  int ls4[6][6][16];
  int ls8[2][6][64];
  explicit Dequant(const h264::ScalingLists& sl) {
    for (int l = 0; l < 6; ++l)
      for (int m = 0; m < 6; ++m)
        for (int k = 0; k < 16; ++k) {
          const int pos = kZigzag4x4[k];
          ls4[l][m][pos] = int(sl.l4[l][k]) * norm_adjust(m, pos >> 2, pos & 3);
        }
    for (int l = 0; l < 2; ++l)
      for (int m = 0; m < 6; ++m)
        for (int k = 0; k < 64; ++k) {
          const int pos = kZigzag8x8[k];
          ls8[l][m][pos] = int(sl.l8[l][k]) * norm_adjust8(m, pos >> 3, pos & 7);
        }
  }
};

const Dequant& dequant_for(const h264::ScalingLists& sl) {
  thread_local h264::ScalingLists last;
  thread_local std::unique_ptr<Dequant> dq;
  if (!dq || std::memcmp(&last, &sl, sizeof sl) != 0) {
    dq = std::make_unique<Dequant>(sl);
    last = sl;
  }
  return *dq;
}

inline int scale4(int c, int ls, int qp) {
  return qp >= 24 ? (c * ls) * (1 << (qp / 6 - 4)) : (c * ls + (1 << (3 - qp / 6))) >> (4 - qp / 6);
}
inline int scale8(int c, int ls, int qp) {
  return qp >= 36 ? (c * ls) * (1 << (qp / 6 - 6)) : (c * ls + (1 << (5 - qp / 6))) >> (6 - qp / 6);
}

constexpr u8 kBPart[23][2] = {{0, 0}, {1, 0}, {2, 0}, {3, 0}, {1, 1}, {1, 1}, {2, 2}, {2, 2},
                              {1, 2}, {1, 2}, {2, 1}, {2, 1}, {1, 3}, {1, 3}, {2, 3}, {2, 3},
                              {3, 1}, {3, 1}, {3, 2}, {3, 2}, {3, 3}, {3, 3}, {0, 0}};
constexpr u8 kBSub[13][2] = {{0, 0}, {1, 0}, {2, 0}, {3, 0}, {1, 1}, {1, 2}, {2, 1},
                             {2, 2}, {3, 1}, {3, 2}, {1, 3}, {2, 3}, {3, 3}};
constexpr int kSubParts[4] = {1, 2, 2, 4};

inline int raster_b8(int blk) { return ((blk >> 3) << 1) | ((blk & 3) >> 1); }
inline u16 b8_blocks(int b8) { return u16(0x33u << ((b8 & 1) * 2 + (b8 >> 1) * 8)); }
inline int clip3i(int lo, int hi, int v) { return v < lo ? lo : (v > hi ? hi : v); }

template <bool kCabac, bool kWrite>
class MbLayer {
  using Bins = std::conditional_t<kWrite, AvcBins<BinEncoder>, AvcBins<BinDecoder>>;

 public:
  MbLayer(MbNeighbours& nb, Picture& pic, const SliceEnv& env, const Dequant& dq)
      : nb_(nb), pic_(pic), env_(env), sh_(*env.sh), pps_(*env.pps), sps_(*env.sps), dq_(dq),
        scan4_(env.field ? kFieldScan4x4 : kZigzag4x4), scan8_(env.field ? kFieldScan8x8 : kZigzag8x8) {
    type_ = sh_.type();
    qp_ = sh_.qp;
    bd_ = sps_.bit_depth_luma;
    qpbd_ = 6 * (sps_.bit_depth_luma - 8);
    qpbdc_ = 6 * (sps_.bit_depth_chroma - 8);
    cf_ = sps_.chroma_format_idc;
    nbc_ = cf_ == 2 ? 8 : 4;
    weighted_ = (type_ == h264::kP && pps_.weighted_pred) || (type_ == h264::kB && pps_.weighted_bipred_idc != 0);
    implicit_ = type_ == h264::kB && pps_.weighted_bipred_idc == 2;
    for (int l = 0; l < 2; ++l) {
      std::fill(std::begin(slot_[l]), std::end(slot_[l]), u8(0xFF));
      if (const auto* lst = env_.list[l])
        for (size_t k = 0; k < lst->size() && k + 1 < std::size(slot_[l]); ++k)
          if ((*lst)[k].slot >= 0) slot_[l][k + 1] = u8((*lst)[k].slot);
    }
    for (int q = 0; q < 52 + qpbd_ && q < int(std::size(qpc_tab_[0])); ++q) {
      qpc_tab_[0][q] = u8(chroma_qp_bd(q - qpbd_, pps_.chroma_qp_index_offset, qpbdc_) + qpbdc_);
      qpc_tab_[1][q] = u8(chroma_qp_bd(q - qpbd_, pps_.second_chroma_qp_index_offset, qpbdc_) + qpbdc_);
    }
    fast_direct_ = !kWrite && type_ == h264::kB && sh_.direct_spatial && sps_.direct_8x8 && !weighted_;
  }

  Bits* br = nullptr;
  BitWriter* bw = nullptr;
  Bins* bins = nullptr;
  cabac::Decoder* cabac = nullptr;
  cabac::Encoder* cenc = nullptr;
  const MbDesc* want = nullptr;
  int prev_qpd_nz = 0;

  int qp() const { return qp_; }

  int ue(u32 v) {
    if constexpr (kWrite) {
      bw->ue(v);
      return int(v);
    } else {
      return int(br->ue());
    }
  }
  int se(int v) {
    if constexpr (kWrite) {
      bw->se(v);
      return v;
    } else {
      return br->se();
    }
  }
  int u(int n, u32 v) {
    if constexpr (kWrite) {
      bw->u(n, v);
      return int(v);
    } else {
      return int(br->u(n));
    }
  }

  static void clear_but_mv(MbState& s) {
    static const MbState z{};
    std::memcpy(static_cast<void*>(&s), &z, offsetof(MbState, mv));
    std::memcpy(static_cast<void*>(&s.mvd), &z.mvd, sizeof(MbState) - offsetof(MbState, mvd));
  }

  bool read_skip_flag(int mb, bool v = false) {
    MbState& s = nb_.at(mb);
    if constexpr (kWrite) s = MbState{};
    else clear_but_mv(s);
    s.slice = u16(env_.slice);
    nb_.begin(mb);
    auto cond = [&](int m) { return m >= 0 && !nb_.at(m).skip ? 1 : 0; };
    const int inc = cond(nb_.mb_at(mb, -1, 0)) + cond(nb_.mb_at(mb, 0, -1));
    return bins->mb_skip(type_ == h264::kB, inc, v) != 0;
  }

  void skip_mb(int mb, bool fresh) {
    MbState& s = nb_.at(mb);
    if (fresh) {
      s = MbState{};
      s.slice = u16(env_.slice);
      nb_.begin(mb);
    }
    s.kind = kSkip;
    s.skip = 1;
    s.qp = u8(qp_ + qpbd_);
    MbResidual res;
    res.luma = 0;
    res.chroma = 0;
    if (type_ == h264::kP) {
      s.ref[0][0] = s.ref[0][1] = s.ref[0][2] = s.ref[0][3] = 0;
      need_ref(0, 0);
      int mv[2];
      nb_.pskip_mv(mb, mv);
      for (auto& v : s.mv[0]) {
        v[0] = i16(mv[0]);
        v[1] = i16(mv[1]);
      }
    } else {
      s.direct16 = 1;
      s.direct8 = 0xF;
      if (fast_direct_) direct16_spatial(mb, s);
      else direct(mb, s, 0xF);
    }
    prev_qpd_nz = 0;
    if (!weighted_ && !kWrite) emit_skip(mb, s);
    else emit(mb, s, res, 0, 0, nullptr);
  }

  void coded_mb(int mb, bool fresh) {
    MbState& s = nb_.at(mb);
    if (fresh) {
      s = MbState{};
      s.slice = u16(env_.slice);
      nb_.begin(mb);
    } else if constexpr (!kWrite) {
      std::memset(static_cast<void*>(s.mv), 0, sizeof s.mv);
    }
    int mbt = read_mb_type(mb, kWrite ? want->mb_type : 0);
    int itype = -1;
    if (type_ == h264::kI) {
      itype = mbt;
    } else if (type_ == h264::kP) {
      VEP_CHECK(mbt <= 30, "bad P mb_type");
      if (mbt >= 5) itype = mbt - 5;
    } else {
      VEP_CHECK(mbt <= 48, "bad B mb_type");
      if (mbt >= 23) itype = mbt - 23;
    }
    VEP_CHECK(itype <= 25, "bad intra mb_type");
    MbResidual res;
    res.luma = 0;
    res.chroma = 0;
    if (itype == 25) {
      pcm_mb(mb, s, res);
      return;
    }
    int cbp = 0, i16_mode = 0;
    const bool intra = itype >= 0;
    bool no_small = true;
    if (itype == 0) {
      if (pps_.transform_8x8_mode) s.t8x8 = u8(read_t8x8(mb, kWrite && want->t8x8));
      s.kind = s.t8x8 ? kI8x8 : kI4x4;
      intra_modes(mb, s);
      s.chroma_mode = u8(read_chroma_mode(mb, kWrite ? want->chroma_mode : 0));
    } else if (itype > 0) {
      s.kind = kI16x16;
      i16_mode = (itype - 1) % 4;
      cbp = (((itype - 1) / 4) % 3) << 4 | (itype >= 13 ? 15 : 0);
      std::fill(std::begin(s.i4), std::end(s.i4), u8(2));
      s.chroma_mode = u8(read_chroma_mode(mb, kWrite ? want->chroma_mode : 0));
      VEP_CHECK(!mono() || (cbp >> 4) == 0, "4:0:0: Intra_16x16 type with chroma coefficients");
    } else {
      s.kind = kInter;
      no_small = inter_pred(mb, s, mbt);
    }
    VEP_CHECK(s.chroma_mode <= 3, "bad intra_chroma_pred_mode");
    if (s.kind != kI16x16) cbp = read_cbp(mb, s, intra, kWrite ? want->cbp : 0);
    s.cbp = u8(cbp);
    if (s.kind == kInter && (cbp & 15) && pps_.transform_8x8_mode && no_small &&
        !(type_ == h264::kB && mbt == 0 && !sps_.direct_8x8))
      s.t8x8 = u8(read_t8x8(mb, kWrite && want->t8x8));
    int qp = qp_;
    if ((cbp & 15) || (cbp >> 4) || s.kind == kI16x16) {
      const int dqp = read_qp_delta(kWrite ? want->qp_delta : 0);
      VEP_CHECK(dqp >= -(26 + qpbd_ / 2) && dqp <= 25 + qpbd_ / 2, "mb_qp_delta out of range");
      qp = (qp + dqp + 52 + 2 * qpbd_) % (52 + qpbd_) - qpbd_;
      prev_qpd_nz = dqp != 0;
    } else {
      prev_qpd_nz = 0;
    }
    qp_ = qp;
    s.qp = u8(qp + qpbd_);
    residual(mb, s, res, cbp & 15, cbp >> 4, qp + qpbd_, intra);
    emit(mb, s, res, i16_mode, s.chroma_mode, nullptr);
// ... 508 lines not shown
    for (int b8 = 0; b8 < 4; ++b8) {
      if (!((mask >> b8) & 1)) continue;
      int r0 = 0;
      for (u16 w = infer ? u16(1u << ((b8 & 1) * 2 + (b8 >> 1) * 8)) : b8_blocks(b8); w; w &= w - 1) {
        const int blk = __builtin_ctz(w);
        const ColMotion::Blk& cb = col->b[col->index(mb, blk)];
        int mvc[2] = {0, 0};
        r0 = 0;
        if (cb.ref >= 0) {
          mvc[0] = cb.mv[0];
          mvc[1] = cb.mv[1];
          r0 = -1;
          for (size_t k = 0; k < l0.size() && r0 < 0; ++k)
            if (l0[k].slot >= 0 && l0[k].uid == cb.pid) r0 = int(k);
          if (r0 < 0) r0 = 0;
        }
        need_ref(0, r0);
        const ListEntry& p0 = l0[size_t(r0)];
        int m0[2], m1[2];
        const int td = clip3i(-128, 127, c1.poc - p0.poc);
        if (td == 0 || p0.long_term) {
          m0[0] = mvc[0];
          m0[1] = mvc[1];
          m1[0] = m1[1] = 0;
        } else {
          const int tb = clip3i(-128, 127, env_.cur_poc - p0.poc);
          const int tx = (16384 + std::abs(td / 2)) / td;
          const int dsf = clip3i(-1024, 1023, (tb * tx + 32) >> 6);
          for (int k = 0; k < 2; ++k) {
            m0[k] = (dsf * mvc[k] + 128) >> 8;
            m1[k] = m0[k] - mvc[k];
          }
        }
        fill(0, b8, blk, clip3i(-32768, 32767, m0[0]), clip3i(-32768, 32767, m0[1]));
        fill(1, b8, blk, clip3i(-32768, 32767, m1[0]), clip3i(-32768, 32767, m1[1]));
      }
      s.ref[0][b8] = i8(r0);
      s.ref[1][b8] = 0;
    }
  }

  void direct16_spatial(int mb, MbState& s) {
    if (!dcol_) {
      VEP_CHECK(env_.list[1] && !env_.list[1]->empty() && (*env_.list[1])[0].slot >= 0,
                "direct prediction without a list-1 reference");
      const ListEntry& c1 = (*env_.list[1])[0];
      VEP_CHECK(c1.col && c1.col->wmbs == nb_.wmbs() && c1.col->hmbs == nb_.hmbs() && c1.col->corners,
                "colocated picture motion missing");
      dcol_ = c1.col;
      dcol_long_ = c1.long_term;
    }
    int ref[2], mvp[2][2];
    nb_.direct_spatial_both(ref, mvp);
    const bool zero = ref[0] < 0 && ref[1] < 0;
    if (zero) ref[0] = ref[1] = 0;
    u32 pv[2];
    for (int l = 0; l < 2; ++l) {
      if (ref[l] >= 0) need_ref(l, ref[l]);
      const bool use = ref[l] >= 0 && !zero;
      pv[l] = use ? (u32(u16(mvp[l][0])) | u32(u16(mvp[l][1])) << 16) : 0u;
      std::memset(s.ref[l], ref[l], 4);
    }
    const ColMotion::Blk* cb = &dcol_->b[size_t(mb) * 4];
    u32 v8[2][4];
    for (int b8 = 0; b8 < 4; ++b8) {
      const bool col_zero = !dcol_long_ && cb[b8].ref == 0 && cb[b8].mv[0] >= -1 && cb[b8].mv[0] <= 1 &&
                            cb[b8].mv[1] >= -1 && cb[b8].mv[1] <= 1;
      for (int l = 0; l < 2; ++l) v8[l][b8] = (ref[l] == 0 && col_zero) ? 0u : pv[l];
    }
    for (int l = 0; l < 2; ++l) {
      u32 row[2][4];
      for (int h = 0; h < 2; ++h) {
        row[h][0] = row[h][1] = v8[l][2 * h];
        row[h][2] = row[h][3] = v8[l][2 * h + 1];
      }
      u8* mv = reinterpret_cast<u8*>(&s.mv[l][0][0]);
      for (int y = 0; y < 4; ++y) std::memcpy(mv + 16 * y, row[y >> 1], 16);
    }
  }

  WpEntry weights(int r0, int r1) { return wp_entry(env_, r0, r1); }

  int cbf_luma_inc(int mb, int blk, bool intra) {
    auto cond = [&](int m, int nblk) -> int {
      if (m < 0) return intra ? 1 : 0;
      const MbState& n = nb_.at(m);
      if (n.kind == kIPcm) return 1;
      if (n.skip) return 0;
      if (!((n.cbp >> raster_b8(nblk)) & 1)) return 0;
      if (n.t8x8) return 1;
      return (n.cbf >> nblk) & 1;
    };
    const int bx = blk & 3, by = blk >> 2;
    const int a = bx > 0 ? cond(mb, blk - 1) : cond(nb_.mb_at(mb, -1, 0), blk + 3);
    const int b = by > 0 ? cond(mb, blk - 4) : cond(nb_.mb_at(mb, 0, -1), blk + 12);
    return a + 2 * b;
  }
  int cbf_dc_inc(int mb, int bit, bool intra) {
    auto cond = [&](int m) -> int {
      if (m < 0) return intra ? 1 : 0;
      const MbState& n = nb_.at(m);
      if (n.kind == kIPcm) return 1;
      if (bit == 0) return n.kind == kI16x16 ? (n.cbf_dc & 1) : 0;
      if (n.skip || (n.cbp >> 4) == 0) return 0;
      return (n.cbf_dc >> bit) & 1;
    };
    return cond(nb_.mb_at(mb, -1, 0)) + 2 * cond(nb_.mb_at(mb, 0, -1));
  }
  int cbf_cac_inc(int mb, int c, int b, bool intra) {
    auto cond = [&](int m, int nb2, bool cur) -> int {
      if (cur) return (nb_.at(mb).cbf_cac[c] >> nb2) & 1;
      if (m < 0) return intra ? 1 : 0;
      const MbState& n = nb_.at(m);
      if (n.kind == kIPcm) return 1;
      if (n.skip || (n.cbp >> 4) != 2) return 0;
      return (n.cbf_cac[c] >> nb2) & 1;
    };
    const int bx = b & 1, by = b >> 1;
    const int a = bx ? cond(mb, b - 1, true) : cond(nb_.mb_at(mb, -1, 0), b + 1, false);
    const int bb = by ? cond(mb, b - 2, true) : cond(nb_.mb_at(mb, 0, -1), b + nbc_ - 2, false);
    return a + 2 * bb;
  }

  int read_block(int cat, int cbf_inc, int nc, int n, int* lv, u8* nzpos, const int* src) {
    if constexpr (kWrite) std::memcpy(lv, src, size_t(n) * sizeof(int));
    (void)src;
    if constexpr (kCabac) {
      (void)nc;
      return bins->residual(cat, cbf_inc, n, lv, nzpos);
    } else {
      (void)cat;
      (void)cbf_inc;
      int t = 0;
      if constexpr (kWrite) {
        for (int k = 0; k < n; ++k)
          if (lv[k]) nzpos[t++] = u8(k);
        write_residual_block(*bw, nc, n, lv);
        return t;
      } else {
        read_residual_block_cb(*br, nc, n, [&](int k, int l) {
          lv[k] = l;
          nzpos[t++] = u8(k);
        });
        return t;
      }
    }
  }

  void residual(int mb, MbState& s, MbResidual& res, int cbp_luma, int cbp_chroma, int qp, bool intra) {
    const int ly = intra ? 0 : 3;
    const int q6 = qp / 6, qm = qp % 6;
    int lv[64];
    u8 nzp[64];
    if (s.kind == kI16x16) {
      const int inc = kCabac ? cbf_dc_inc(mb, 0, true) : 0;
      const int nc = kCabac ? 0 : nb_.nc_luma(mb, 0);
      int dcy[16] = {};
      const int tdc = read_block(kCatLumaDc, inc, nc, 16, lv, nzp, kWrite ? want->dc : nullptr);
      if (tdc > 0) {
        s.cbf_dc |= 1;
        int c[16] = {};
        for (int j = 0; j < tdc; ++j) c[scan4_[nzp[j]]] = lv[nzp[j]];
        hadamard4x4(c);
        const int ls = dq_.ls4[ly][qm][0];
        for (int k = 0; k < 16; ++k)
          dcy[k] = qp >= 36 ? c[k] * ls * (1 << (q6 - 6)) : (c[k] * ls + (1 << (5 - q6))) >> (6 - q6);
      }
      for (int idx = 0; idx < 16; ++idx) {
        const int r = blk_to_raster(idx);
        i16* d = res.blk[r];
        bool nz = dcy[r] != 0;
        std::memset(d, 0, 16 * sizeof(i16));
        d[0] = sat16(dcy[r]);
        if (cbp_luma) {
          const int binc = kCabac ? cbf_luma_inc(mb, r, true) : 0;
          const int bnc = kCabac ? 0 : nb_.nc_luma(mb, r);
          const int tc = read_block(kCatLumaAc, binc, bnc, 15, lv, nzp, kWrite ? want->ac[r] : nullptr);
          for (int j = 0; j < tc; ++j) {
            const int k = nzp[j];
            const int pos = scan4_[k + 1];
            const int v = scale4(lv[k], dq_.ls4[ly][qm][pos], qp);
            d[pos] = sat16(v);
            nz |= v != 0;
          }
          s.tc[r] = u8(tc);
          if (tc) s.cbf |= u16(1u << r);
        }
        if (nz) res.luma |= u16(1u << r);
      }
    } else if (s.t8x8) {
      res.t8 = true;
      const int l8 = intra ? 0 : 1;
      for (int b8 = 0; b8 < 4; ++b8) {
        if (!((cbp_luma >> b8) & 1)) continue;
        i16* d = res.b8[b8];
        std::memset(d, 0, 64 * sizeof(i16));
        bool nz = false;
        int total = 0;
        auto put = [&](int k, int level) {
          const int pos = scan8_[k];
          const int v = scale8(level, dq_.ls8[l8][qm][pos], qp);
          d[pos] = sat16(v);
          nz |= v != 0;
        };
        if constexpr (kCabac) {
          total = read_block(kCatLuma8x8, -1, 0, 64, lv, nzp, kWrite ? want->l8[b8] : nullptr);
          for (int j = 0; j < total; ++j) put(nzp[j], lv[nzp[j]]);
          for (u16 w = b8_blocks(b8); w; w &= w - 1) s.tc[__builtin_ctz(w)] = u8(std::min(total, 16));
        } else {
          for (int i4 = 0; i4 < 4; ++i4) {
            const int r = blk_to_raster(b8 * 4 + i4);
            int part[16] = {};
            if constexpr (kWrite)
              for (int k = 0; k < 16; ++k) part[k] = want->l8[b8][4 * k + i4];
            const int tc = read_block(kCatLuma4x4, 0, nb_.nc_luma(mb, r), 16, lv, nzp, part);
            s.tc[r] = u8(tc);
            total += tc;
            for (int j = 0; j < tc; ++j) put(4 * nzp[j] + i4, lv[nzp[j]]);
          }
        }
        if (total) {
          s.cbf |= b8_blocks(b8);
          nz8_ |= b8_blocks(b8);
        }
        if (nz) res.luma |= b8_blocks(b8);
      }
    } else {
      for (int idx = 0; idx < 16; ++idx) {
        const int r = blk_to_raster(idx);
        if (!((cbp_luma >> (idx >> 2)) & 1)) continue;
        const int binc = kCabac ? cbf_luma_inc(mb, r, intra) : 0;
        const int bnc = kCabac ? 0 : nb_.nc_luma(mb, r);
        const int tc = read_block(kCatLuma4x4, binc, bnc, 16, lv, nzp, kWrite ? want->ac[r] : nullptr);
        s.tc[r] = u8(tc);
        if (!tc) continue;
        s.cbf |= u16(1u << r);
        i16* d = res.blk[r];
        std::memset(d, 0, 16 * sizeof(i16));
        bool nz = false;
        for (int j = 0; j < tc; ++j) {
          const int k = nzp[j];
          const int pos = scan4_[k];
          const int v = scale4(lv[k], dq_.ls4[ly][qm][pos], qp);
          d[pos] = sat16(v);
          nz |= v != 0;
        }
        if (nz) res.luma |= u16(1u << r);
      }
    }
    if (cbp_chroma) {
      const int qpc[2] = {chroma_qp_bd(qp - qpbd_, pps_.chroma_qp_index_offset, qpbdc_) + qpbdc_,
                          chroma_qp_bd(qp - qpbd_, pps_.second_chroma_qp_index_offset, qpbdc_) + qpbdc_};
      const int nbc = nbc_;
      int dcv[2][8] = {};
      for (int c = 0; c < 2; ++c) {
        const int inc = kCabac ? cbf_dc_inc(mb, 1 + c, intra) : 0;
        int v8[8];
        const int t = read_block(kCatChromaDc, inc, cf_ == 2 ? -2 : -1, nbc, v8, nzp, kWrite ? want->cdc[c] : nullptr);
        if (t > 0) {
          s.cbf_dc |= u8(2 << c);
          int u[8] = {0, 0, 0, 0, 0, 0, 0, 0};
          for (int j = 0; j < t; ++j) u[nzp[j]] = v8[nzp[j]];
          if (cf_ == 2) {
            const int qpdc = qpc[c] + 3;
            chroma422_dc(u, qpdc, dq_.ls4[ly + 1 + c][qpdc % 6][0], dcv[c]);
          } else {
            const int f[4] = {u[0] + u[1] + u[2] + u[3], u[0] - u[1] + u[2] - u[3], u[0] + u[1] - u[2] - u[3],
                              u[0] - u[1] - u[2] + u[3]};
            const int ls = dq_.ls4[ly + 1 + c][qpc[c] % 6][0];
            for (int b = 0; b < 4; ++b) dcv[c][b] = ((f[b] * ls) * (1 << (qpc[c] / 6))) >> 5;
          }
        }
      }
      for (int c = 0; c < 2; ++c) {
        const int lc = ly + 1 + c;
        for (int b = 0; b < nbc; ++b) {
          i16* d = res.blk[16 + c * nbc + b];
          bool nz = dcv[c][b] != 0;
          std::memset(d, 0, 16 * sizeof(i16));
          d[0] = sat16(dcv[c][b]);
          if (cbp_chroma & 2) {
            const int binc = kCabac ? cbf_cac_inc(mb, c, b, intra) : 0;
            const int bnc = kCabac ? 0 : nb_.nc_chroma(mb, c, b, nbc);
            const int tc = read_block(kCatChromaAc, binc, bnc, 15, lv, nzp, kWrite ? want->cac[c][b] : nullptr);
            s.tcc[c][b] = u8(tc);
            if (tc) s.cbf_cac[c] |= u8(1u << b);
            for (int j = 0; j < tc; ++j) {
              const int k = nzp[j];
              const int pos = scan4_[k + 1];
              const int v = scale4(lv[k], dq_.ls4[lc][qpc[c] % 6][pos], qpc[c]);
              d[pos] = sat16(v);
              nz |= v != 0;
            }
          }
          if (nz) res.chroma |= u16(1u << (c * nbc + b));
        }
      }
    }
    if constexpr (!kCabac && !kWrite) VEP_CHECK(!br->overrun(), "slice data overrun");
  }

  void emit(int mb, const MbState& s, const MbResidual& res, int i16_mode, int chroma_mode, const u8* pcm) {
    MbRec m{};
    m.kind = s.kind;
    m.qp = u8(s.kind == kIPcm ? qpbd_ : s.qp);
    VEP_CHECK(m.qp < std::size(qpc_tab_[0]), "macroblock QP out of range");
    m.qpc = qpc_tab_[0][m.qp];
    m.qpc2 = qpc_tab_[1][m.qp];
    m.i16_mode = u8(i16_mode);
    m.chroma_mode = u8(chroma_mode);
    m.dbk = u8((sh_.disable_deblocking == 1 ? 1 : 0) | (sh_.disable_deblocking == 2 ? 2 : 0));
    m.alpha_off = i8(sh_.alpha_off);
    m.beta_off = i8(sh_.beta_off);
    m.slice = s.slice;
    m.flags = s.t8x8 && s.kind != kI8x8 ? kMbT8x8 : 0;
    if (s.kind == kI8x8) m.flags = kMbT8x8;
    bool l1 = false;
    const bool intra = is_intra(s.kind);
    for (int k = 0; k < 4; ++k) {
      m.ref[k] = intra ? u8(0xFF) : slot_[0][s.ref[0][k] + 1];
      m.ref1[k] = intra ? u8(0xFF) : slot_[1][s.ref[1][k] + 1];
      l1 |= !intra && s.ref[1][k] >= 0;
    }
    if (l1) m.flags |= kMbL1;
    u16 nz = 0;
    if (s.t8x8) {
      nz = nz8_;
      if (!kCabac)
        for (int b8 = 0; b8 < 4; ++b8) {
          bool any = false;
          for (u16 w = b8_blocks(b8); w; w &= w - 1) any |= s.tc[__builtin_ctz(w)] != 0;
          if (any) nz |= b8_blocks(b8);
        }
    } else {
      nz = s.cbf;
    }
    nz8_ = 0;
    m.nz = nz;
    if (s.kind == kI4x4)
      for (int r = 0; r < 16; ++r) m.i4[r >> 1] |= u8(s.i4[r] << ((r & 1) * 4));
    if (s.kind == kI8x8)
      for (int b8 = 0; b8 < 4; ++b8) m.i4[b8 >> 1] |= u8(s.i4[(b8 & 1) * 2 + (b8 >> 1) * 8] << ((b8 & 1) * 4));
    WpEntry wp[4];
    bool use_wp = false;
    if (weighted_ && !is_intra(s.kind)) {
      for (int k = 0; k < 4; ++k) {
        wp[k] = weights(s.ref[0][k], s.ref[1][k]);
        const WpEntry& e = wp[k];
        for (int c = 0; c < 3; ++c)
          use_wp |= !(e.lwd[c] == 0 && e.w0[c] == 1 && e.w1[c] == 1 && e.o[c] == 0) &&
                    !(e.w0[c] == (1 << e.lwd[c]) && e.w1[c] == (1 << e.lwd[c]) && e.o[c] == 0);
      }
      if (use_wp) m.flags |= kMbWp;
    }
    store_mb(pic_, mb, m, s, &res, pcm, use_wp ? wp : nullptr);
  }

  void emit_skip(int mb, const MbState& s) {
    MbRec m{};
    m.kind = kSkip;
    m.qp = s.qp;
    VEP_CHECK(m.qp < std::size(qpc_tab_[0]), "macroblock QP out of range");
    m.qpc = qpc_tab_[0][m.qp];
    m.qpc2 = qpc_tab_[1][m.qp];
    m.dbk = u8((sh_.disable_deblocking == 1 ? 1 : 0) | (sh_.disable_deblocking == 2 ? 2 : 0));
    m.alpha_off = i8(sh_.alpha_off);
    m.beta_off = i8(sh_.beta_off);
    m.slice = s.slice;
    bool l1 = false;
    for (int k = 0; k < 4; ++k) {
      m.ref[k] = slot_[0][s.ref[0][k] + 1];
      m.ref1[k] = slot_[1][s.ref[1][k] + 1];
      l1 |= s.ref[1][k] >= 0;
    }
    m.flags = l1 ? kMbL1 : 0;
    nz8_ = 0;
    store_skip_mb(pic_, mb, m, s);
  }

  MbNeighbours& nb_;
  Picture& pic_;
  const SliceEnv& env_;
  const SliceHdr& sh_;
  const h264::Pps& pps_;
  const h264::Sps& sps_;
  const Dequant& dq_;
  const u8* scan4_;
  const u8* scan8_;
  int type_ = 0;
  int qp_ = 26;
  bool weighted_ = false, implicit_ = false;
  u16 nz8_ = 0;
  u8 slot_[2][33];
  u8 qpc_tab_[2][96];
  bool fast_direct_ = false;
  const ColMotion* dcol_ = nullptr;
  bool dcol_long_ = false;
};

}

WpEntry wp_entry(const SliceEnv& env, int r0, int r1) {
  const SliceHdr& sh = *env.sh;
  const bool implicit = sh.type() == h264::kB && env.pps->weighted_bipred_idc == 2;
  WpEntry e{};
  for (int c = 0; c < 3; ++c) {
    e.w0[c] = e.w1[c] = 1;
    e.o[c] = 0;
    e.lwd[c] = 0;
  }
  if (implicit) {
    if (r0 < 0 || r1 < 0) return e;
    const ListEntry& p0 = (*env.list[0])[size_t(r0)];
    const ListEntry& p1 = (*env.list[1])[size_t(r1)];
    int w0 = 32, w1 = 32;
    const int td = clip3i(-128, 127, p1.poc - p0.poc);
    if (td != 0 && !p0.long_term && !p1.long_term) {
      const int tb = clip3i(-128, 127, env.cur_poc - p0.poc);
      const int tx = (16384 + std::abs(td / 2)) / td;
      const int dsf = clip3i(-1024, 1023, (tb * tx + 32) >> 6);
      if ((dsf >> 2) >= -64 && (dsf >> 2) <= 128) {
        w1 = dsf >> 2;
        w0 = 64 - w1;
      }
    }
    for (int c = 0; c < 3; ++c) {
      e.w0[c] = i16(w0);
      e.w1[c] = i16(w1);
      e.lwd[c] = 5;
    }
    return e;
  }
  for (int c = 0; c < 3; ++c) e.lwd[c] = u8(c == 0 ? sh.luma_lwd : sh.chroma_lwd);
  int o0[3] = {0, 0, 0}, o1[3] = {0, 0, 0};
  if (r0 >= 0) {
    const auto& w = sh.wt[0][size_t(r0)];
    for (int c = 0; c < 3; ++c) {
      e.w0[c] = w.w[c];
      o0[c] = w.o[c];
    }
  }
  if (r1 >= 0) {
    const auto& w = sh.wt[1][size_t(r1)];
    for (int c = 0; c < 3; ++c) {
      e.w1[c] = w.w[c];
      o1[c] = w.o[c];
    }
  }
  for (int c = 0; c < 3; ++c) {
    const int sc = 1 << ((c == 0 ? env.sps->bit_depth_luma : env.sps->bit_depth_chroma) - 8);
    o0[c] *= sc;
    o1[c] *= sc;
    e.o[c] = i16(r0 >= 0 && r1 >= 0 ? (o0[c] + o1[c] + 1) >> 1 : (r0 >= 0 ? o0[c] : o1[c]));
  }
  return e;
}

void decode_slice_generic(MbNeighbours& nb, Picture& pic, const SliceEnv& env, const u8* data, size_t n,
                          size_t bitpos) {
  const SliceHdr& sh = *env.sh;
  const Dequant& dq = dequant_for(env.scaling);
  const int total = pic.nmbs();
  int mb = sh.first_mb;
  VEP_CHECK(mb < total, "first_mb_in_slice past end of picture");
  if (env.pps->cabac) {
    if (sh.type() != h264::kI && sh.cabac_init_idc != 0)
      throw UnsupportedStream("CABAC cabac_init_idc " + std::to_string(sh.cabac_init_idc) + " is not supported");
    const size_t start = (bitpos + 7) >> 3;
    VEP_CHECK(start <= n, "slice data overrun");
    cabac::Ctx ctx[kCabacCtx];
    cabac_init_contexts(ctx, sh.type() == h264::kI ? -1 : 0, std::max(0, sh.qp));
    cabac::Decoder dec(data, n, start);
    BinDecoder bd{dec, ctx};
    AvcBins<BinDecoder> bins{bd};
    MbLayer<true, false> L(nb, pic, env, dq);
    L.bins = &bins;
    L.cabac = &dec;
    L.data = data;
    L.data_n = n;
    for (;;) {
      VEP_CHECK(mb < total, "macroblock address past end of picture");
      if (sh.type() != h264::kI && L.read_skip_flag(mb)) L.skip_mb(mb, false);
      else L.coded_mb(mb, sh.type() == h264::kI);
      ++mb;
      if (bins.end_of_slice(false)) {
        cabac::bins_decoded().fetch_add(dec.bins(), std::memory_order_relaxed);
        break;
      }
      VEP_CHECK(dec.bitpos() <= n * 8 + 16, "slice data overrun");
    }
    return;
  }
  Bits br(data, n, bitpos);
  const size_t stop = BitReader(data, n).stop_bit_pos();
  MbLayer<false, false> L(nb, pic, env, dq);
  L.br = &br;
  bool more = true;
  while (more) {
    if (sh.type() != h264::kI) {
      const u32 run = br.ue();
      VEP_CHECK(u32(total - mb) >= run, "mb_skip_run past end of picture");
      for (u32 k = 0; k < run; ++k) L.skip_mb(mb++, true);
      if (run > 0) {
        more = br.pos() < stop;
        if (!more) break;
      }
    }
    VEP_CHECK(mb < total, "macroblock address past end of picture");
    L.coded_mb(mb, true);
    VEP_CHECK(!br.overrun(), "slice data overrun");
    more = br.pos() < stop;
    ++mb;
  }
}


struct SliceWriter::Impl {
  const SliceEnv& env;
  BitWriter& bw;
  Dequant dq;
  bool cabac;
  bool is_i;
  int run = 0;
  bool first = true;
  cabac::Ctx ctx[kCabacCtx];
  std::unique_ptr<cabac::Encoder> enc;
  std::unique_ptr<BinEncoder> be;
  std::unique_ptr<AvcBins<BinEncoder>> bins;
  std::unique_ptr<MbLayer<true, true>> lc;
  std::unique_ptr<MbLayer<false, true>> lv;
  Impl(MbNeighbours& nb, Picture& pic, const SliceEnv& e, BitWriter& w)
      : env(e), bw(w), dq(e.scaling), cabac(e.pps->cabac), is_i(e.sh->type() == h264::kI) {
    if (cabac) {
      while (!bw.byte_aligned()) bw.u1(1);
      cabac_init_contexts(ctx, is_i ? -1 : 0, std::max(0, e.sh->qp));
      enc = std::make_unique<cabac::Encoder>(bw.buf());
      be = std::make_unique<BinEncoder>(BinEncoder{*enc, ctx});
      bins = std::make_unique<AvcBins<BinEncoder>>(AvcBins<BinEncoder>{*be});
      lc = std::make_unique<MbLayer<true, true>>(nb, pic, env, dq);
      lc->bins = bins.get();
      lc->cenc = enc.get();
    } else {
      lv = std::make_unique<MbLayer<false, true>>(nb, pic, env, dq);
      lv->bw = &bw;
    }
  }
};

// ... 48 lines not shown
```

### csrc/vep/avc_recon.h

```cpp
#pragma once

#include "common.h"

#if defined(__HIPCC__)
#include <hip/hip_runtime.h>
#define VEP_HD __host__ __device__ inline
#else
#define VEP_HD inline
#endif
#if defined(__HIP_DEVICE_COMPILE__)
#define VEP_CONST __constant__
#else
#define VEP_CONST
#endif

namespace vep::avc {

using i16 = int16_t;
using i8 = int8_t;

enum MbKind : u8 { kSkip = 0, kInter = 1, kI4x4 = 2, kI16x16 = 3, kIPcm = 4, kI8x8 = 5 };
VEP_HD bool is_intra(u8 k) { return k >= kI4x4; }
VEP_HD bool is_wave_intra(u8 k) { return k == kI4x4 || k == kI16x16 || k == kI8x8; }

constexpr u8 kMbT8x8 = 1;
constexpr u8 kMbL1 = 2;
constexpr u8 kMbWp = 4;
constexpr u8 kMbMv8x8 = 8;
constexpr u8 kMbMv16 = 16;

struct MbRec {
  u8 kind;
  u8 qp;
  u8 qpc;
  u8 qpc2;
  u8 i16_mode;
  u8 chroma_mode;
  u8 dbk;
  u8 flags;
  u16 nz;
  u16 luma_coded;
  i8 alpha_off;
  i8 beta_off;
  u16 slice;
  u16 chroma_coded;
  u16 pad1;
  u8 ref[4];
  u8 ref1[4];
  u32 coef;
  u32 mv;
  u8 i4[8];
  u32 res;
  u32 wp;
  u32 pad2;
};
static_assert(sizeof(MbRec) == 56, "MbRec layout");
constexpr u32 kNoRes = 0xFFFFFFFFu;

VEP_HD int mv_per_list(u8 flags) { return (flags & kMbMv16) ? 2 : ((flags & kMbMv8x8) ? 8 : 32); }
VEP_HD int byte_at(const u8* a, int i) {
  u32 w;
  __builtin_memcpy(&w, a, 4);
  return int((w >> (8 * i)) & 0xFFu);
}

VEP_HD int mv_sub(u8 flags, int list, int blk) {
  const int k = (flags & kMbMv16) ? 0 : ((flags & kMbMv8x8) ? 2 * (((blk >> 3) << 1) | ((blk & 3) >> 1)) : 2 * blk);
  return list * mv_per_list(flags) + k;
}

struct WpEntry {
  i16 w0[3], w1[3];
  i16 o[3];
  u8 lwd[3];
  u8 pad[11];
};
static_assert(sizeof(WpEntry) == 32, "WpEntry layout");

VEP_HD int wp_sample(int p0, int p1, bool has0, bool has1, const WpEntry* w, int c, int bd = 8) {
  if (!w) return has0 && has1 ? (p0 + p1 + 1) >> 1 : (has0 ? p0 : p1);
  const int lwd = w->lwd[c], mx = (1 << bd) - 1;
  if (has0 && has1) {
    const int v = ((p0 * w->w0[c] + p1 * w->w1[c] + (1 << lwd)) >> (lwd + 1)) + w->o[c];
    return v < 0 ? 0 : (v > mx ? mx : v);
  }
  const int p = has0 ? p0 : p1, ww = has0 ? w->w0[c] : w->w1[c];
  const int v = lwd >= 1 ? ((p * ww + (1 << (lwd - 1))) >> lwd) + w->o[c] : p * ww + w->o[c];
  return v < 0 ? 0 : (v > mx ? mx : v);
}

constexpr int kDenseCoefs = 512;
VEP_HD int coef_words(const MbRec& m) {
  return __builtin_popcount(u32(m.luma_coded)) + __builtin_popcount(u32(m.chroma_coded));
}
VEP_HD int coef_word_base(const MbRec& m, int j) {
  const u32 lc = m.luma_coded;
  const int nl = __builtin_popcount(lc);
  if (j >= nl) {
    u32 cc = m.chroma_coded;
    for (int k = j - nl; k > 0; --k) cc &= cc - 1;
    return 256 + 16 * __builtin_ctz(cc);
  }
  if (m.flags & kMbT8x8) {
    const u32 qm = (lc & 1u) | ((lc >> 1) & 2u) | ((lc >> 6) & 4u) | ((lc >> 7) & 8u);
    u32 q = qm;
    for (int k = j >> 2; k > 0; --k) q &= q - 1;
    return 64 * __builtin_ctz(q) + 16 * (j & 3);
  }
  u32 w = lc;
  for (int k = j; k > 0; --k) w &= w - 1;
  return 16 * __builtin_ctz(w);
}
inline void expand_coefs(const i16* pool, const MbRec& m, i16* dense) {
  for (int i = 0; i < kDenseCoefs; ++i) dense[i] = 0;
  const int nw = coef_words(m);
  const i16* v = pool + m.coef + nw;
  for (int j = 0; j < nw; ++j) {
    const u32 mask = u16(pool[m.coef + j]);
    i16* d = dense + coef_word_base(m, j);
    for (u32 b = mask; b; b &= b - 1) d[__builtin_ctz(b)] = *v++;
  }
}
inline u32 coef_values(const i16* pool, const MbRec& m) {
  u32 n = 0;
  for (int j = 0, nw = coef_words(m); j < nw; ++j) n += u32(__builtin_popcount(u32(u16(pool[m.coef + j]))));
  return n;
}

VEP_HD int i4_mode(const MbRec& m, int blk) { return (m.i4[blk >> 1] >> ((blk & 1) * 4)) & 15; }

VEP_HD int blk_to_raster(int idx) {
  return ((idx >> 3) << 3) | (((idx >> 1) & 1) << 2) | (((idx >> 2) & 1) << 1) | (idx & 1);
}
VEP_HD int raster_to_blk(int r) {
  const int bx = r & 3, by = r >> 2;
  return ((by >> 1) << 3) | ((bx >> 1) << 2) | ((by & 1) << 1) | (bx & 1);
}

VEP_CONST static const u8 kNormAdjust[6][3] = {
    {10, 16, 13}, {11, 18, 14}, {13, 20, 16}, {14, 23, 18}, {16, 25, 20}, {18, 29, 23}};

VEP_HD int norm_adjust(int m, int i, int j) {
  const int cls = ((i & 1) == 0 && (j & 1) == 0) ? 0 : ((i & 1) && (j & 1)) ? 1 : 2;
  return kNormAdjust[m][cls];
}

VEP_CONST static const u8 kChromaQp[52] = {
    0,  1,  2,  3,  4,  5,  6,  7,  8,  9,  10, 11, 12, 13, 14, 15, 16, 17,
    18, 19, 20, 21, 22, 23, 24, 25, 26, 27, 28, 29, 29, 30, 31, 32, 32, 33,
    34, 34, 35, 35, 36, 36, 37, 37, 37, 38, 38, 38, 39, 39, 39, 39};

VEP_HD int chroma_qp(int qpy, int offset) {
  int q = qpy + offset;
  q = q < 0 ? 0 : q > 51 ? 51 : q;
  return kChromaQp[q];
}
VEP_HD int chroma_qp_bd(int qpy, int offset, int qpbd_c) {
  int q = qpy + offset;
  q = q < -qpbd_c ? -qpbd_c : q > 51 ? 51 : q;
  return q < 0 ? q : kChromaQp[q];
}

VEP_CONST static const u8 kZigzag4x4[16] = {0, 1, 4, 8, 5, 2, 3, 6, 9, 12, 13, 10, 7, 11, 14, 15};
VEP_CONST static const u8 kFieldScan4x4[16] = {0, 4, 1, 8, 12, 5, 9, 13, 2, 6, 10, 14, 3, 7, 11, 15};

VEP_CONST static const u8 kAlpha[52] = {
    0,  0,  0,  0,  0,  0,  0,  0,  0,  0,  0,  0,   0,   0,   0,   0,   4,   4,
    5,  6,  7,  8,  9,  10, 12, 13, 15, 17, 20, 22,  25,  28,  32,  36,  40,  45,
    50, 56, 63, 71, 80, 90, 101, 113, 127, 144, 162, 182, 203, 226, 255, 255};
VEP_CONST static const u8 kBeta[52] = {
    0, 0, 0, 0, 0, 0, 0, 0, 0, 0, 0, 0, 0,  0,  0,  0,  2,  2,  2,  3,  3,  3,  3,  4,  4,  4,
    6, 6, 7, 7, 8, 8, 9, 9, 10, 10, 11, 11, 12, 12, 13, 13, 14, 14, 15, 15, 16, 16, 17, 17, 18, 18};
VEP_CONST static const u8 kTc0[52][3] = {
    {0, 0, 0},   {0, 0, 0},   {0, 0, 0},   {0, 0, 0},   {0, 0, 0},    {0, 0, 0},    {0, 0, 0},
    {0, 0, 0},   {0, 0, 0},   {0, 0, 0},   {0, 0, 0},   {0, 0, 0},    {0, 0, 0},    {0, 0, 0},
    {0, 0, 0},   {0, 0, 0},   {0, 0, 0},   {0, 0, 1},   {0, 0, 1},    {0, 0, 1},    {0, 0, 1},
    {0, 1, 1},   {0, 1, 1},   {1, 1, 1},   {1, 1, 1},   {1, 1, 1},    {1, 1, 1},    {1, 1, 2},
    {1, 1, 2},   {1, 1, 2},   {1, 1, 2},   {1, 2, 3},   {1, 2, 3},    {2, 2, 3},    {2, 2, 4},
    {2, 3, 4},   {2, 3, 4},   {3, 3, 5},   {3, 4, 6},   {3, 4, 6},    {4, 5, 7},    {4, 5, 8},
    {4, 6, 9},   {5, 7, 10},  {6, 8, 11},  {6, 8, 13},  {7, 10, 14},  {8, 11, 16},  {9, 12, 18},
    {10, 13, 20}, {11, 15, 23}, {13, 17, 25}};

VEP_HD int clip1(int x, int bd = 8) { return x < 0 ? 0 : (x > (1 << bd) - 1 ? (1 << bd) - 1 : x); }
VEP_HD int clip3(int lo, int hi, int x) { return x < lo ? lo : (x > hi ? hi : x); }
VEP_HD int iabs(int x) { return x < 0 ? -x : x; }
VEP_HD int imin(int a, int b) { return a < b ? a : b; }
VEP_HD int imax(int a, int b) { return a > b ? a : b; }

VEP_HD int dequant4x4(int c, int qp, int i, int j) {
  const int ls = 16 * norm_adjust(qp % 6, i, j);
  if (qp >= 24) return c * ls * (1 << (qp / 6 - 4));
  return (c * ls + (1 << (3 - qp / 6))) >> (4 - qp / 6);
}

VEP_HD void idct4x4(const i16* d, int* r) {
  int f[16];
  for (int i = 0; i < 4; ++i) {
    const int d0 = d[i * 4], d1 = d[i * 4 + 1], d2 = d[i * 4 + 2], d3 = d[i * 4 + 3];
    const int e0 = d0 + d2, e1 = d0 - d2, e2 = (d1 >> 1) - d3, e3 = d1 + (d3 >> 1);
    f[i * 4] = e0 + e3;
    f[i * 4 + 1] = e1 + e2;
    f[i * 4 + 2] = e1 - e2;
    f[i * 4 + 3] = e0 - e3;
  }
  for (int j = 0; j < 4; ++j) {
    const int f0 = f[j], f1 = f[4 + j], f2 = f[8 + j], f3 = f[12 + j];
    const int g0 = f0 + f2, g1 = f0 - f2, g2 = (f1 >> 1) - f3, g3 = f1 + (f3 >> 1);
    r[j] = (g0 + g3 + 32) >> 6;
    r[4 + j] = (g1 + g2 + 32) >> 6;
    r[8 + j] = (g1 - g2 + 32) >> 6;
    r[12 + j] = (g0 - g3 + 32) >> 6;
  }
}

VEP_HD int idct4x4_at(const i16* d, int i, int j) {
  int f[4];
  for (int k = 0; k < 4; ++k) {
    const int d0 = d[k * 4], d1 = d[k * 4 + 1], d2 = d[k * 4 + 2], d3 = d[k * 4 + 3];
    const int e0 = d0 + d2, e1 = d0 - d2, e2 = (d1 >> 1) - d3, e3 = d1 + (d3 >> 1);
    f[k] = j == 0 ? e0 + e3 : j == 1 ? e1 + e2 : j == 2 ? e1 - e2 : e0 - e3;
  }
  const int g0 = f[0] + f[2], g1 = f[0] - f[2], g2 = (f[1] >> 1) - f[3], g3 = f[1] + (f[3] >> 1);
  const int h = i == 0 ? g0 + g3 : i == 1 ? g1 + g2 : i == 2 ? g1 - g2 : g0 - g3;
  return (h + 32) >> 6;
}

VEP_CONST static const u8 kZigzag8x8[64] = {
    0,  1,  8,  16, 9,  2,  3,  10, 17, 24, 32, 25, 18, 11, 4,  5,  12, 19, 26, 33, 40, 48,
    41, 34, 27, 20, 13, 6,  7,  14, 21, 28, 35, 42, 49, 56, 57, 50, 43, 36, 29, 22, 15, 23,
    30, 37, 44, 51, 58, 59, 52, 45, 38, 31, 39, 46, 53, 60, 61, 54, 47, 55, 62, 63};

VEP_CONST static const u8 kFieldScan8x8[64] = {
    0,  8,  16, 1,  9,  24, 32, 17, 2,  25, 40, 48, 56, 33, 10, 3,  18, 41, 49, 57, 26, 11,
    4,  19, 34, 42, 50, 58, 27, 12, 5,  20, 35, 43, 51, 59, 28, 13, 6,  21, 36, 44, 52, 60,
    29, 14, 22, 37, 45, 53, 61, 30, 7,  15, 38, 46, 54, 62, 23, 31, 39, 47, 55, 63};

VEP_CONST static const u8 kNormAdjust8[6][6] = {{20, 18, 32, 19, 25, 24}, {22, 19, 35, 21, 28, 26},
                                                {26, 23, 42, 24, 33, 31}, {28, 25, 45, 26, 35, 33},
                                                {32, 28, 51, 30, 40, 38}, {36, 32, 58, 34, 46, 43}};
VEP_HD int norm_adjust8(int m, int i, int j) {
  int cls;
  if ((i & 3) == 0 && (j & 3) == 0) cls = 0;
  else if ((i & 1) && (j & 1)) cls = 1;
  else if ((i & 3) == 2 && (j & 3) == 2) cls = 2;
  else if (((i & 3) == 0 && (j & 1)) || ((i & 1) && (j & 3) == 0)) cls = 3;
  else if (((i & 3) == 0 && (j & 3) == 2) || ((i & 3) == 2 && (j & 3) == 0)) cls = 4;
  else cls = 5;
  return kNormAdjust8[m][cls];
}

VEP_HD void idct8_1d(int* x) {
  const int a0 = x[0] + x[4], a4 = x[0] - x[4];
  const int a2 = (x[2] >> 1) - x[6], a6 = x[2] + (x[6] >> 1);
  const int b0 = a0 + a6, b2 = a4 + a2, b4 = a4 - a2, b6 = a0 - a6;
  const int a1 = -x[3] + x[5] - x[7] - (x[7] >> 1);
  const int a3 = x[1] + x[7] - x[3] - (x[3] >> 1);
  const int a5 = -x[1] + x[7] + x[5] + (x[5] >> 1);
  const int a7 = x[3] + x[5] + x[1] + (x[1] >> 1);
  const int b1 = a1 + (a7 >> 2), b7 = a7 - (a1 >> 2), b3 = a3 + (a5 >> 2), b5 = (a3 >> 2) - a5;
  x[0] = b0 + b7;
  x[1] = b2 + b5;
  x[2] = b4 + b3;
  x[3] = b6 + b1;
  x[4] = b6 - b1;
  x[5] = b4 - b3;
  x[6] = b2 - b5;
  x[7] = b0 - b7;
}

VEP_HD void idct8x8(const i16* d, int* r) {
  int t[64];
  for (int i = 0; i < 8; ++i) {
    int x[8];
    for (int k = 0; k < 8; ++k) x[k] = d[i * 8 + k];
    idct8_1d(x);
    for (int k = 0; k < 8; ++k) t[i * 8 + k] = x[k];
  }
  for (int j = 0; j < 8; ++j) {
    int x[8];
    for (int k = 0; k < 8; ++k) x[k] = t[k * 8 + j];
    idct8_1d(x);
    for (int k = 0; k < 8; ++k) r[k * 8 + j] = (x[k] + 32) >> 6;
  }
}

template <class TF, class LF>
VEP_HD int intra8x8_filter_at(TF T, LF L, bool has_top, bool has_left, bool has_tl, int k) {
  if (k == 0) {
    if (!has_tl) return 128;
    if (has_top && has_left) return (T(0) + 2 * T(-1) + L(0) + 2) >> 2;
    if (has_top) return (3 * T(-1) + T(0) + 2) >> 2;
    if (has_left) return (3 * T(-1) + L(0) + 2) >> 2;
    return T(-1);
  }
  if (k <= 16) {
    if (!has_top) return 128;
    const int x = k - 1;
    if (x == 0) return has_tl ? (T(-1) + 2 * T(0) + T(1) + 2) >> 2 : (3 * T(0) + T(1) + 2) >> 2;
    if (x == 15) return (T(14) + 3 * T(15) + 2) >> 2;
    return (T(x - 1) + 2 * T(x) + T(x + 1) + 2) >> 2;
  }
  if (!has_left) return 128;
  const int y = k - 17;
  if (y == 0) return has_tl ? (T(-1) + 2 * L(0) + L(1) + 2) >> 2 : (3 * L(0) + L(1) + 2) >> 2;
  if (y == 7) return (L(6) + 3 * L(7) + 2) >> 2;
  return (L(y - 1) + 2 * L(y) + L(y + 1) + 2) >> 2;
}

template <class TF, class LF>
VEP_HD void intra8x8_filter(TF T, LF L, bool has_top, bool has_left, bool has_tl, int* f) {
  for (int k = 0; k < 25; ++k) f[k] = intra8x8_filter_at(T, L, has_top, has_left, has_tl, k);
}

template <class TF, class LF>
VEP_HD int intra8x8_pred_g(TF T, LF L, bool has_top, bool has_left, int mode, int x, int y, int bd = 8) {
  switch (mode) {
    case 0: return T(x);
    case 1: return L(y);
    case 2: {
      int s = 0;
      if (has_top && has_left) {
        for (int k = 0; k < 8; ++k) s += T(k) + L(k);
        return (s + 8) >> 4;
      }
      if (has_left) {
        for (int k = 0; k < 8; ++k) s += L(k);
        return (s + 4) >> 3;
      }
      if (has_top) {
        for (int k = 0; k < 8; ++k) s += T(k);
        return (s + 4) >> 3;
      }
      return 1 << (bd - 1);
    }
    case 3:
      if (x == 7 && y == 7) return (T(14) + 3 * T(15) + 2) >> 2;
      return (T(x + y) + 2 * T(x + y + 1) + T(x + y + 2) + 2) >> 2;
    case 4:
      if (x > y) return (T(x - y - 2) + 2 * T(x - y - 1) + T(x - y) + 2) >> 2;
      if (x < y) return (L(y - x - 2) + 2 * L(y - x - 1) + L(y - x) + 2) >> 2;
      return (T(0) + 2 * T(-1) + L(0) + 2) >> 2;
    case 5: {
      const int z = 2 * x - y;
      if (z >= 0 && (z & 1) == 0) return (T(x - (y >> 1) - 1) + T(x - (y >> 1)) + 1) >> 1;
      if (z >= 0) return (T(x - (y >> 1) - 2) + 2 * T(x - (y >> 1) - 1) + T(x - (y >> 1)) + 2) >> 2;
      if (z == -1) return (L(0) + 2 * L(-1) + T(0) + 2) >> 2;
      return (L(y - 2 * x - 1) + 2 * L(y - 2 * x - 2) + L(y - 2 * x - 3) + 2) >> 2;
    }
    case 6: {
      const int z = 2 * y - x;
      if (z >= 0 && (z & 1) == 0) return (L(y - (x >> 1) - 1) + L(y - (x >> 1)) + 1) >> 1;
      if (z >= 0) return (L(y - (x >> 1) - 2) + 2 * L(y - (x >> 1) - 1) + L(y - (x >> 1)) + 2) >> 2;
      if (z == -1) return (L(0) + 2 * L(-1) + T(0) + 2) >> 2;
      return (T(x - 2 * y - 1) + 2 * T(x - 2 * y - 2) + T(x - 2 * y - 3) + 2) >> 2;
    }
    case 7:
      if ((y & 1) == 0) return (T(x + (y >> 1)) + T(x + (y >> 1) + 1) + 1) >> 1;
      return (T(x + (y >> 1)) + 2 * T(x + (y >> 1) + 1) + T(x + (y >> 1) + 2) + 2) >> 2;
    default: {
      const int z = x + 2 * y;
      if (z > 13) return L(7);
      if (z == 13) return (L(6) + 3 * L(7) + 2) >> 2;
      if ((z & 1) == 0) return (L(y + (x >> 1)) + L(y + (x >> 1) + 1) + 1) >> 1;
      return (L(y + (x >> 1)) + 2 * L(y + (x >> 1) + 1) + L(y + (x >> 1) + 2) + 2) >> 2;
    }
  }
}

constexpr u32 kTap8Const = 1u << 30, kTap8Dc = 1u << 31;
VEP_HD u32 pack_tap8(int i0, int i1, int i2, int w0, int w1, int w2, int add, int shift) {
  return u32(i0) | u32(i1) << 5 | u32(i2) << 10 | u32(w0) << 15 | u32(w1) << 17 | u32(w2) << 19 |
         u32(add) << 21 | u32(shift) << 23;
}
VEP_HD int eval_tap8(u32 t, int s0, int s1, int s2) {
  return (int((t >> 15) & 3) * s0 + int((t >> 17) & 3) * s1 + int((t >> 19) & 3) * s2 + int((t >> 21) & 3)) >>
         int((t >> 23) & 3);
}
VEP_HD u32 intra8x8_pred_tap(int mode, int x, int y) {
  auto T = [](int i) { return 1 + i; };
  auto L = [](int j) { return j < 0 ? 0 : 17 + j; };
  auto t3 = [](int a, int b, int c) { return pack_tap8(a, b, c, 1, 2, 1, 2, 2); };
  auto t2 = [](int a, int b) { return pack_tap8(a, b, 0, 1, 1, 0, 1, 1); };
  auto cp = [](int a) { return pack_tap8(a, a, a, 1, 2, 1, 2, 2); };
  switch (mode) {
    case 0: return cp(T(x));
    case 1: return cp(L(y));
    case 2: return kTap8Dc;
    case 3:
      if (x == 7 && y == 7) return pack_tap8(T(14), T(15), 0, 1, 3, 0, 2, 2);
      return t3(T(x + y), T(x + y + 1), T(x + y + 2));
    case 4:
      if (x > y) return t3(T(x - y - 2), T(x - y - 1), T(x - y));
      if (x < y) return t3(L(y - x - 2), L(y - x - 1), L(y - x));
      return t3(T(0), T(-1), L(0));
    case 5: {
      const int z = 2 * x - y;
      if (z >= 0 && (z & 1) == 0) return t2(T(x - (y >> 1) - 1), T(x - (y >> 1)));
      if (z >= 0) return t3(T(x - (y >> 1) - 2), T(x - (y >> 1) - 1), T(x - (y >> 1)));
      if (z == -1) return t3(L(0), L(-1), T(0));
      return t3(L(y - 2 * x - 1), L(y - 2 * x - 2), L(y - 2 * x - 3));
    }
// ... 592 lines not shown
```

### csrc/vep/gpu_avc.hip

```cpp
#define VEP_KERNEL_SOURCE 1
#include "avc_recon.h"
#include "gpu.h"

namespace vep::gpu {

using avc::MbRec;
using avc::kDenseCoefs;

namespace {

constexpr int kIntraWaves = kAvcDbkWgRows;
constexpr int kIntraXgWords = 8;
constexpr int kIntraLine = 32;
constexpr int kIntraLineCols = 240;
constexpr u32 kSpinLimit = 1u << 24;

__device__ inline const MbRec& rec(const AvcDesc& d, int mb) {
  return static_cast<const MbRec*>(d.mbs)[mb];
}


__device__ inline void wave_sync() {
  __builtin_amdgcn_fence(__ATOMIC_RELEASE, "wavefront");
  __builtin_amdgcn_wave_barrier();
  __builtin_amdgcn_fence(__ATOMIC_ACQUIRE, "wavefront");
}

#define VEP_GLOBAL __attribute__((address_space(1)))
#define VEP_LDS __attribute__((address_space(3)))
__device__ inline u32 gld1(const void* p) { return *(const VEP_GLOBAL u8*)(p); }
__device__ inline u32 gld4(const void* p) { return *(const VEP_GLOBAL u32*)(p); }
typedef u32 vu2 __attribute__((ext_vector_type(2)));
typedef u32 vu4 __attribute__((ext_vector_type(4)));
__device__ inline uint2 gld8(const void* p) {
  const vu2 v = *(const VEP_GLOBAL vu2*)(p);
  return make_uint2(v.x, v.y);
}
__device__ inline uint4 gld16(const void* p) {
  const vu4 v = *(const VEP_GLOBAL vu4*)(p);
  return make_uint4(v.x, v.y, v.z, v.w);
}
__device__ inline void gst4(void* p, u32 v) { *(VEP_GLOBAL u32*)(p) = v; }


__device__ inline void expand_coefs_wave(const AvcDesc& d, const MbRec& m, int lane, i16* D) {
  if (lane < kDenseCoefs / 8) reinterpret_cast<uint4*>(D)[lane] = make_uint4(0, 0, 0, 0);
  const int nw = avc::coef_words(m);
  const VEP_DEV i16* pool = d.coefs + m.coef;
  u32 mask = 0;
  int base = 0;
  if (lane < nw) {
    mask = u32(u16(pool[lane]));
    base = avc::coef_word_base(m, lane);
  }
  const int cnt = __popc(mask);
  int incl = cnt;
#pragma unroll
  for (int o = 1; o < 32; o <<= 1) {
    const int t = __shfl_up(incl, o);
    if (lane >= o) incl += t;
  }
  wave_sync();
  if (lane < nw) {
    const VEP_DEV i16* v = pool + nw + (incl - cnt);
    for (u32 b = mask; b; b &= b - 1) D[base + __ffs(int(b)) - 1] = *v++;
  }
  wave_sync();
}

constexpr int kT8Pitch = 9, kT8Block = 8 * kT8Pitch, kT8Ints = 4 * kT8Block;
static_assert(kT8Ints >= 256, "the transpose buffer also holds the 16x16 raster result");
__device__ inline void luma8_residual(const i16* D, const MbRec& m, int lane, int* T) {
  if (lane < 32) {
    const int q = lane >> 3, i = lane & 7;
    int v[8] = {0, 0, 0, 0, 0, 0, 0, 0};
    if ((m.luma_coded >> ((q & 1) * 2 + (q >> 1) * 8)) & 1) {
      const uint4 w = *reinterpret_cast<const uint4*>(D + q * 64 + i * 8);
      const u32 ws[4] = {w.x, w.y, w.z, w.w};
#pragma unroll
      for (int k = 0; k < 4; ++k) {
        v[2 * k] = int(i16(ws[k] & 0xffff));
        v[2 * k + 1] = int(i16(ws[k] >> 16));
      }
      avc::idct8_1d(v);
    }
#pragma unroll
    for (int k = 0; k < 8; ++k) T[q * kT8Block + i * kT8Pitch + k] = v[k];
  }
  wave_sync();
  int c[8];
  const int q = (lane >> 3) & 3, j = lane & 7;
  if (lane < 32) {
#pragma unroll
    for (int k = 0; k < 8; ++k) c[k] = T[q * kT8Block + k * kT8Pitch + j];
    avc::idct8_1d(c);
  }
  wave_sync();
  if (lane < 32) {
#pragma unroll
    for (int k = 0; k < 8; ++k) T[((q >> 1) * 8 + k) * 16 + (q & 1) * 8 + j] = (c[k] + 32) >> 6;
  }
  wave_sync();
}

template <class P, int CF>
__device__ inline void inter_mb(const AvcDesc& d, const MbRec& m, int mb, int lane, int* T, i16* D, bool t8) {
  constexpr int CH = CF == 2 ? 16 : 8;
  constexpr int CS = 8 * CH;
  constexpr int NCL = 2 * CS / 64;
  constexpr int NB = CF == 2 ? 8 : 4;
  const int x = lane & 15, y0 = lane >> 4;
  const int W = d.wmbs, wpx = W * 16, hpx = d.hmbs * 16, pitch = wpx;
  const int mx = mb % W, my = mb / W;
  const int bd = sizeof(P) == 1 ? 8 : d.bd;
  VEP_DEV P* ty = reinterpret_cast<VEP_DEV P*>(d.y + d.slot_y * u64(d.target));
  VEP_DEV P* tuv = reinterpret_cast<VEP_DEV P*>(d.uv + d.slot_uv * u64(d.target));
  auto yref = [&](int s) { return reinterpret_cast<const VEP_DEV P*>(d.y + d.slot_y * u64(s)); };
  auto uvref = [&](int s) { return reinterpret_cast<const VEP_DEV P*>(d.uv + d.slot_uv * u64(s)); };
  constexpr bool kCheck = sizeof(P) == 2 || CF == 2;
  if (kCheck) {
    const u32 need = m.kind == avc::kIPcm ? u32((256 + 2 * CS) * sizeof(P) / 2) : 0u;
    if (u64(m.coef) + need > u64(d.ncoef)) {
      atomicOr(d.err, 0x4000u);
      return;
    }
  }
  if (m.kind == avc::kIPcm) {
    const VEP_DEV P* s = reinterpret_cast<const VEP_DEV P*>(d.coefs + m.coef);
#pragma unroll
    for (int k = 0; k < 4; ++k) ty[size_t(my * 16 + y0 + 4 * k) * pitch + mx * 16 + x] = s[(y0 + 4 * k) * 16 + x];
#pragma unroll
    for (int k = 0; k < NCL; ++k) {
      const int t = lane + 64 * k, cc = t / CS, cq = t % CS, cx = cq & 7, cy = cq >> 3;
      tuv[size_t(my * CH + cy) * pitch + (mx * 8 + cx) * 2 + cc] = s[256 + t];
    }
    return;
  }
  const i16* mvb = d.mvs + size_t(m.mv);
  const bool l1 = (m.flags & avc::kMbL1) != 0;
  const avc::WpEntry* wpp =
      (m.flags & avc::kMbWp) ? static_cast<const avc::WpEntry*>(d.wps) + m.wp : nullptr;
  int v[4];
#pragma unroll
  for (int k = 0; k < 4; ++k) {
    const int y = y0 + 4 * k, blk = k * 4 + (x >> 2), b8 = ((y >> 3) << 1) | (x >> 3);
    const int s0 = avc::byte_at(m.ref, b8), s1 = l1 ? avc::byte_at(m.ref1, b8) : 0xFF;
    int p0 = 0, p1 = 0;
    if (s0 != 0xFF) {
      const i16* v0 = mvb + avc::mv_sub(m.flags, 0, blk);
      p0 = avc::luma_qpel(yref(s0), pitch, wpx, hpx, mx * 16 + x + (v0[0] >> 2),
                          my * 16 + y + (v0[1] >> 2), v0[0] & 3, v0[1] & 3, bd);
    }
    if (s1 != 0xFF) {
      const i16* v1 = mvb + avc::mv_sub(m.flags, 1, blk);
      p1 = avc::luma_qpel(yref(s1), pitch, wpx, hpx, mx * 16 + x + (v1[0] >> 2),
                          my * 16 + y + (v1[1] >> 2), v1[0] & 3, v1[1] & 3, bd);
    }
    v[k] = avc::wp_sample(p0, p1, s0 != 0xFF, s1 != 0xFF, wpp ? wpp + b8 : nullptr, 0, bd);
  }
  if (m.luma_coded | m.chroma_coded) expand_coefs_wave(d, m, lane, D);
  if (t8) luma8_residual(D, m, lane, T);
#pragma unroll
  for (int k = 0; k < 4; ++k) {
    const int y = y0 + 4 * k, blk = k * 4 + (x >> 2);
    int o = v[k];
    if (t8) o += T[y * 16 + x];
    else if ((m.luma_coded >> blk) & 1) o += avc::idct4x4_at(D + 16 * blk, y & 3, x & 3);
    ty[size_t(my * 16 + y) * pitch + mx * 16 + x] = P(avc::clip1(o, bd));
  }
  int u[NCL];
  const int chp = CF == 2 ? hpx : hpx / 2;
#pragma unroll
  for (int k = 0; k < NCL; ++k) {
    const int t = lane + 64 * k, cc = t / CS, cq = t % CS, cx = cq & 7, cy = cq >> 3;
    const int ly = CF == 2 ? cy : 2 * cy;
    const int r = (ly >> 2) * 4 + (cx >> 1), b8 = ((ly >> 3) << 1) | (cx >> 2);
    const int s0 = avc::byte_at(m.ref, b8), s1 = l1 ? avc::byte_at(m.ref1, b8) : 0xFF;
    int p0 = 0, p1 = 0, ix, fx, iy, fy;
    if (s0 != 0xFF) {
      const i16* v0 = mvb + avc::mv_sub(m.flags, 0, r);
      const int vy = v0[1] + (d.field ? 2 * ((d.field == 2) - (s0 & 1)) : 0);
      avc::chroma_mv(v0[0], vy, CF, ix, fx, iy, fy);
      p0 = avc::chroma_epel(uvref(s0), pitch, wpx / 2, chp, cc, mx * 8 + cx + ix, my * CH + cy + iy, fx, fy);
    }
    if (s1 != 0xFF) {
      const i16* v1 = mvb + avc::mv_sub(m.flags, 1, r);
      const int vy = v1[1] + (d.field ? 2 * ((d.field == 2) - (s1 & 1)) : 0);
      avc::chroma_mv(v1[0], vy, CF, ix, fx, iy, fy);
      p1 = avc::chroma_epel(uvref(s1), pitch, wpx / 2, chp, cc, mx * 8 + cx + ix, my * CH + cy + iy, fx, fy);
    }
    u[k] = avc::wp_sample(p0, p1, s0 != 0xFF, s1 != 0xFF, wpp ? wpp + b8 : nullptr, 1 + cc, bd);
  }
#pragma unroll
  for (int k = 0; k < NCL; ++k) {
    const int t = lane + 64 * k, cc = t / CS, cq = t % CS, cx = cq & 7, cy = cq >> 3;
    const int kb = cc * NB + (cy >> 2) * 2 + (cx >> 2);
    int o = u[k];
    if ((m.chroma_coded >> kb) & 1) o += avc::idct4x4_at(D + 256 + 16 * kb, cy & 3, cx & 3);
    tuv[size_t(my * CH + cy) * pitch + (mx * 8 + cx) * 2 + cc] = P(avc::clip1(o, bd));
  }
}

__global__ __launch_bounds__(256) void avc_inter_kernel(const AvcDesc* __restrict__ descs, int n,
                                                         int total) {
  __shared__ int lres[4][kT8Ints];
  __shared__ alignas(16) i16 lcoef[4][kDenseCoefs];
  const int wv = int(threadIdx.x) >> 6;
  const int g = __builtin_amdgcn_readfirstlane(int(blockIdx.x) * 4 + wv);
  if (g >= total) return;
  int lo = 0, hi = n - 1;
  while (lo < hi) {
    const int mid = (lo + hi + 1) >> 1;
    if (descs[mid].mb_begin <= g) lo = mid;
    else hi = mid - 1;
  }
  const AvcDesc d = descs[lo];
  const int mb = g - d.mb_begin;
  const MbRec m = rec(d, mb);
// ... 1073 lines not shown
```

Measured before the change: 8445.

## Store raw AVC coefficient levels and dequantize them on the GPU during expansion

The CPU parser now keeps raw scan-order levels with per-group masks instead of dequantizing and zigzag-placing coefficients into dense blocks. The GPU coefficient-expansion kernel, and the host expand_coefs, perform the dequant and zigzag placement when an MB carries the new kMbLevels flag. This moves per-coefficient dequant arithmetic and dense memsets off the CPU parse threads, which are likely the bottleneck at 256 streams. In exchange it adds GPU-side per-coefficient work, keeps a fallback path for levels that do not fit in 16 bits, is restricted to 8-bit 4:2:0 content with flat scaling lists, and is on by default through an environment variable.

```diff
diff --git a/csrc/bindings.cpp b/csrc/bindings.cpp
--- a/csrc/bindings.cpp
+++ b/csrc/bindings.cpp
@@ -1013,6 +1013,107 @@
       }
     }
     return std::make_pair(bad_avc, bad_hevc);
+  });
+  m.def("set_avc_coef_levels", &avc::set_coef_levels, py::arg("on"),
+        "Override VEP_AVC_COEF_LEVELS for the slices parsed from now on (tests, A/B)");
+  m.def("avc_coef_levels_enabled", &avc::coef_levels_enabled);
+  m.def("avc_coef_levels_case", [](const std::string& kind, int qp, int qpc, int qpc2, const std::vector<int>& luma,
+                                   const std::vector<int>& luma_dc, const std::vector<int>& chroma,
+                                   const std::vector<int>& chroma_dc, bool descending) {
+    VEP_CHECK(kind == "4x4" || kind == "8x8" || kind == "i16", "kind: 4x4, 8x8 or i16");
+    VEP_CHECK(luma.size() == 256 && luma_dc.size() == 16 && chroma.size() == 128 && chroma_dc.size() == 8,
+              "luma 256, luma_dc 16, chroma 128, chroma_dc 8 entries");
+    VEP_CHECK(qp >= 0 && qp <= 51 && qpc >= 0 && qpc <= 51 && qpc2 >= 0 && qpc2 <= 51, "QP out of range");
+    const bool t8 = kind == "8x8", i16x16 = kind == "i16";
+    avc::MbResidual res;
+    res.t8 = t8;
+    res.levels = true;
+    std::memset(res.lmask, 0, sizeof res.lmask);
+    std::vector<i16> want(avc::kDenseCoefs, 0), got(avc::kDenseCoefs, 0);
+    int lv[64];
+    u8 nzp[64];
+    auto stage = [&](int at, const int* src, int first, int n, int dc, int q, bool b8) {
+      int n0 = 0, tc = 0;
+      if (first && dc != 0) {
+        want[size_t(at)] = res.lvl[at] = avc::sat16(dc);
+        res.lmask[at >> 4] = 1;
+        n0 = 1;
+      }
+      for (int k = first; k < n; ++k) {
+        if (!src[k]) continue;
+        lv[k - first] = src[k];
+        nzp[tc++] = u8(k - first);
+        if (b8) {
+          const int pos = avc::kZigzag8x8[k];
+          want[size_t(at + pos)] = avc::sat16(avc::scale8(src[k], 16 * avc::norm_adjust8(q % 6, pos >> 3, pos & 7), q));
+        } else {
+          const int pos = avc::kZigzag4x4[k];
+          want[size_t(at + pos)] = avc::sat16(avc::scale4(src[k], 16 * avc::norm_adjust(q % 6, pos >> 2, pos & 3), q));
+        }
+      }
+      if (descending) std::reverse(nzp, nzp + tc);
+      res.put_levels(at, n0, lv, nzp, tc, first, descending);
+      return tc != 0 || n0 != 0;
+    };
+    if (t8) {
+      for (int q = 0; q < 4; ++q)
+        if (stage(64 * q, luma.data() + 64 * q, 0, 64, 0, qp, true)) res.luma |= u16(0x33u << ((q & 1) * 2 + (q >> 1) * 8));
+    } else {
+      for (int r = 0; r < 16; ++r)
+        if (stage(16 * r, luma.data() + 16 * r, i16x16 ? 1 : 0, 16, luma_dc[size_t(r)], qp, false)) res.luma |= u16(1u << r);
+    }
+    for (int k = 0; k < 8; ++k)
+      if (stage(256 + 16 * k, chroma.data() + 16 * k, 1, 16, chroma_dc[size_t(k)], k < 4 ? qpc : qpc2, false))
+        res.chroma |= u16(1u << k);
+    const int wide = res.nwide;
+    if (wide) avc::levels_to_blocks(res, i16x16, qp, qpc, qpc2);
+    avc::Picture pic;
+    pic.wmbs = pic.hmbs = 1;
+    pic.mbs.resize(1);
+    avc::MbRec rec{};
+    rec.kind = i16x16 ? avc::kI16x16 : (t8 ? avc::kI8x8 : avc::kI4x4);
+    rec.flags = t8 ? u8(avc::kMbT8x8) : u8(0);
+    rec.qp = u8(qp);
+    rec.qpc = u8(qpc);
+    rec.qpc2 = u8(qpc2);
+    avc::MbState s;
+    avc::store_mb(pic, 0, rec, s, &res, nullptr);
+    const avc::MbRec& out = pic.mbs[0];
+    avc::expand_coefs(pic.coefs.data(), out, got.data());
+    py::dict d;
+    d["levels"] = (out.flags & avc::kMbLevels) != 0;
+    d["wide"] = wide;
+    d["got"] = got;
+    d["want"] = want;
+    d["pool"] = pic.coefs.size();
+    d["words"] = avc::coef_words(out);
+    d["values"] = avc::coef_values(pic.coefs.data(), out);
+    d["luma_coded"] = int(out.luma_coded);
+    d["chroma_coded"] = int(out.chroma_coded);
+    d["masks"] = std::vector<int>(pic.coefs.begin(), pic.coefs.begin() + avc::coef_words(out));
+    return d;
+  }, py::arg("kind"), py::arg("qp"), py::arg("qpc"), py::arg("qpc2"), py::arg("luma"), py::arg("luma_dc"),
+     py::arg("chroma"), py::arg("chroma_dc"), py::arg("descending") = false);
+  m.def("avc_level_stats", [](const std::vector<std::shared_ptr<AccessUnit>>& aus) {
+    std::vector<std::tuple<int, int, int>> out;
+    py::gil_scoped_release r;
+    avc::Decoder dec;
+    for (const auto& au : aus) {
+      size_t nal = 0;
+      do {
+        auto p = dec.parse(*au, 0, &nal);
+        if (!p) continue;
+        int coded = 0, lev = 0, slices = 0;
+        for (const avc::MbRec& m : p->mbs) {
+          slices = std::max(slices, int(m.slice) + 1);
+          if (m.kind == avc::kIPcm || !(m.luma_coded | m.chroma_coded)) continue;
+          ++coded;
+          lev += (m.flags & avc::kMbLevels) != 0;
+        }
+        out.emplace_back(coded, lev, slices);
+      } while (nal < au->nals.size());
+    }
+    return out;
   });
   m.def("avc_parse_seconds", [](const std::vector<std::shared_ptr<AccessUnit>>& aus, int reps) {
     py::gil_scoped_release r;
diff --git a/csrc/vep/avc.cpp b/csrc/vep/avc.cpp
--- a/csrc/vep/avc.cpp
+++ b/csrc/vep/avc.cpp
@@ -4,6 +4,8 @@
 
 #include <algorithm>
 #include <array>
+#include <atomic>
+#include <cstdlib>
 
 #include "avc_cavlc.h"
 #include "avc_internal.h"
@@ -1141,7 +1143,34 @@
                    q >= 24 ? 0 : 4 - q / 6};
     };
     const auto dl = scaler(qp);
+    const bool lev = coef_levels_enabled() && pic_.bd == 8;
+    if (lev) {
+      res.levels = true;
+      std::memset(res.lmask, 0, sizeof res.lmask);
+    }
+    int lv[16];
+    u8 nzp[16];
+    auto stage_block = [&](int at, int nc, int start, int max_coeff, int dcv) {
+      if (start && dcv != 0) {
+        res.lvl[at] = sat16(dcv);
+        res.lmask[at >> 4] = 1;
+      }
+      int t = 0;
+      const int tc = read_residual_block_cb(br, nc, max_coeff, [&](int k, int l) {
+        lv[k] = l;
+        nzp[t++] = u8(k);
+      });
+      res.put_levels(at, start && dcv != 0 ? 1 : 0, lv, nzp, tc, start, true);
+      return tc;
+    };
     auto luma_block = [&](int r, int start, int max_coeff, int dcv) {
+      if (lev) {
+        const int tc = stage_block(16 * r, ncl(r), start, max_coeff, dcv);
+        s.tc[r] = u8(tc);
+        ncl_[((r >> 2) + 1) * 5 + (r & 3) + 1] = u8(tc);
+        if (tc || dcv != 0) res.luma |= u16(1u << r);
+        return;
+      }
       i16* d = res.blk[r];
       std::memset(d, 0, 16 * sizeof(i16));
       bool nz = dcv != 0;
@@ -1172,9 +1201,14 @@
         if (cbp_luma) {
           luma_block(r, 1, 15, dcy[r]);
         } else if (dcy[r] != 0) {
-          i16* d = res.blk[r];
-          std::memset(d, 0, 16 * sizeof(i16));
-          d[0] = sat16(dcy[r]);
+          if (lev) {
+            res.lvl[16 * r] = sat16(dcy[r]);
+            res.lmask[r] = 1;
+          } else {
+            i16* d = res.blk[r];
+            std::memset(d, 0, 16 * sizeof(i16));
+            d[0] = sat16(dcy[r]);
+          }
           res.luma |= u16(1u << r);
         }
       }
@@ -1198,7 +1232,18 @@
         for (int b = 0; b < 4; ++b) {
           i16* d = res.blk[16 + c * 4 + b];
           bool nz = dcv[c][b] != 0;
-          if (cbp_chroma & 2) {
+          if (lev) {
+            const int at = 256 + 16 * (c * 4 + b);
+            if (cbp_chroma & 2) {
+              const int tc = stage_block(at, ncc(c, b), 1, 15, dcv[c][b]);
+              s.tcc[c][b] = u8(tc);
+              ncc_[c][((b >> 1) + 1) * 3 + (b & 1) + 1] = u8(tc);
+              nz |= tc != 0;
+            } else if (nz) {
+              res.lvl[at] = sat16(dcv[c][b]);
+              res.lmask[at >> 4] = 1;
+            }
+          } else if (cbp_chroma & 2) {
             std::memset(d, 0, 16 * sizeof(i16));
             d[0] = sat16(dcv[c][b]);
             const int tc = read_residual_block_cb(br, ncc(c, b), 15, [&](int k, int l) {
@@ -1217,6 +1262,10 @@
         }
     }
     VEP_CHECK(!br.overrun(), "slice data overrun");
+    if (lev && res.nwide) {
+      const int qpc = chroma_qp(qp, sc_.pps.chroma_qp_index_offset);
+      levels_to_blocks(res, intra16, qp, qpc, qpc);
+    }
   }
 
   void emit(int mb, const MbState& s, const MbResidual& res, int i16_mode, int chroma_mode) {
@@ -1693,6 +1742,7 @@
   VEP_CHECK(size_t(m.coef) + nw <= ncoef, "coefficient masks outside the pool");
   VEP_CHECK(written || size_t(m.coef) + nw + coef_values(p.coefs.data(), m) <= ncoef, "coefficients outside the pool");
   VEP_CHECK(m.chroma_mode <= 3 && m.i16_mode <= 3, "intra prediction mode out of range");
+  VEP_CHECK(!(m.flags & kMbLevels) || (p.bd == 8 && p.cf == 1), "coefficient levels outside 8-bit 4:2:0");
   if (m.flags & kMbT8x8)
     for (int q = 0; q < 4; ++q) {
       const u32 g = (u32(m.luma_coded) >> ((q & 1) * 2 + (q >> 1) * 8)) & 0x33u;
@@ -1726,6 +1776,7 @@
   if (m.kind != kIPcm) {
     ok &= size_t(m.coef) + size_t(coef_words(m)) <= ncoef;
     ok &= (m.chroma_mode <= 3) & (m.i16_mode <= 3);
+    ok &= !(m.flags & kMbLevels) | ((p.bd == 8) & (p.cf == 1));
     if (m.flags & kMbT8x8)
       for (int q = 0; q < 4; ++q) {
         const u32 g = (u32(m.luma_coded) >> ((q & 1) * 2 + (q >> 1) * 8)) & 0x33u;
@@ -2087,6 +2138,54 @@
   stream_words(dst, &m, sizeof(MbRec));
 }
 
+static std::atomic<int> g_coef_levels{-1};
+
+bool coef_levels_enabled() {
+  int v = g_coef_levels.load(std::memory_order_relaxed);
+  if (v < 0) {
+    const char* e = std::getenv("VEP_AVC_COEF_LEVELS");
+    v = !(e && e[0] == '0');
+    g_coef_levels.store(v, std::memory_order_relaxed);
+  }
+  return v != 0;
+}
+void set_coef_levels(bool on) { g_coef_levels.store(on ? 1 : 0, std::memory_order_relaxed); }
+
+void levels_to_blocks(MbResidual& res, bool i16x16, int qp, int qpc, int qpc2) {
+  auto level = [&](int idx) {
+    for (int k = 0; k < res.nwide; ++k)
+      if (res.wide_at[k] == idx) return res.wide[k];
+    return int(res.lvl[idx]);
+  };
+  if (res.t8) {
+    for (int q = 0; q < 4; ++q) {
+      if (!((res.luma >> ((q & 1) * 2 + (q >> 1) * 8)) & 1)) continue;
+      i16* d = res.b8[q];
+      std::memset(d, 0, 64 * sizeof(i16));
+      int n = 64 * q;
+      for (int w = 0; w < 4; ++w)
+        for (u32 b = res.lmask[4 * q + w]; b; b &= b - 1) {
+          const int pos = kZigzag8x8[16 * w + __builtin_ctz(b)];
+          d[pos] = sat16(scale8(level(n++), 16 * norm_adjust8(qp % 6, pos >> 3, pos & 7), qp));
+        }
+    }
+  }
+  for (int g = res.t8 ? 16 : 0; g < 24; ++g) {
+    if (!((g < 16 ? res.luma >> g : res.chroma >> (g - 16)) & 1)) continue;
+    const bool dc = g < 16 ? i16x16 : true;
+    const int q = g < 16 ? qp : (g < 20 ? qpc : qpc2);
+    i16* d = res.blk[g];
+    std::memset(d, 0, 16 * sizeof(i16));
+    int n = 16 * g;
+    for (u32 b = res.lmask[g]; b; b &= b - 1) {
+      const int i = __builtin_ctz(b), pos = kZigzag4x4[i];
+      d[pos] = dc && i == 0 ? res.lvl[n++] : sat16(dequant4x4(level(n++), q, pos >> 2, pos & 3));
+    }
+  }
+  res.levels = false;
+  res.nwide = 0;
+}
+
 void store_skip_mb(Picture& pic, int mb, MbRec& m, const MbState& s) {
   m.coef = u32(pic.coefs.size());
   m.luma_coded = 0;
@@ -2119,6 +2218,42 @@
     const size_t o = pic.coefs.size(), nb = pic.bd > 8 ? 2 * ns : ns;
     pic.coefs.resize(o + nb / 2);
     std::memcpy(pic.coefs.data() + o, pcm, nb);
+  } else if (res && res->levels && (res->luma | res->chroma)) {
+    m.luma_coded = res->luma;
+    m.chroma_coded = res->chroma;
+    m.flags |= u8(kMbLevels | (res->t8 ? kMbT8x8 : 0));
+    int at[24];
+    int ng = 0, nv = 0;
+    if (res->t8) {
+      for (int q = 0; q < 4; ++q)
+        if ((res->luma >> ((q & 1) * 2 + (q >> 1) * 8)) & 1)
+          for (int w = 0; w < 4; ++w) at[ng++] = 64 * q + 16 * w;
+    } else {
+      for (u32 w = res->luma; w; w &= w - 1) at[ng++] = 16 * __builtin_ctz(w);
+    }
+    for (u32 w = res->chroma; w; w &= w - 1) at[ng++] = 256 + 16 * __builtin_ctz(w);
+    u16 mask[24];
+    for (int g = 0; g < ng; ++g) {
+      mask[g] = res->lmask[at[g] >> 4];
+      nv += __builtin_popcount(mask[g]);
+    }
+    const size_t o = pic.coefs.size();
+    i16* out = pic.coefs.extend(size_t(ng + nv) + 16);
+    std::memcpy(out, mask, size_t(ng) * sizeof(u16));
+    i16* v = out + ng;
+    for (int g = 0; g < ng; ++g) {
+      if (res->t8 && at[g] < 256) {
+        if (at[g] & 63) continue;
+        const int n = __builtin_popcount(mask[g]) + __builtin_popcount(mask[g + 1]) +
+                      __builtin_popcount(mask[g + 2]) + __builtin_popcount(mask[g + 3]);
+        std::memcpy(v, res->lvl + at[g], size_t(n) * sizeof(i16));
+        v += n;
+      } else {
+        std::memcpy(v, res->lvl + at[g], 16 * sizeof(i16));
+        v += __builtin_popcount(mask[g]);
+      }
+    }
+    pic.coefs.resize(o + size_t(ng + nv));
   } else if (res && (res->luma | res->chroma)) {
     m.luma_coded = res->luma;
     m.chroma_coded = res->chroma;
diff --git a/csrc/vep/avc.h b/csrc/vep/avc.h
--- a/csrc/vep/avc.h
+++ b/csrc/vep/avc.h
@@ -501,7 +501,45 @@
   u16 luma = 0;
   u16 chroma = 0;
   bool t8 = false;
-};
+  bool levels = false;
+  u16 lmask[24];
+  i16 lvl[kDenseCoefs - 128];
+  static constexpr int kMaxWide = 384;
+  int nwide = 0;
+  int wide[kMaxWide];
+  u16 wide_at[kMaxWide];
+
+  void put_levels(int at, int n0, const int* lv, const u8* nzp, int tc, int shift, bool descending) {
+    i16* v = lvl + at + n0;
+    u64 m = 0;
+    u32 high = 0;
+    const int j0 = descending ? tc - 1 : 0, dj = descending ? -1 : 1;
+    for (int j = 0; j < tc; ++j) {
+      const int k = nzp[j0 + dj * j], l = lv[k];
+      v[j] = i16(l);
+      m |= u64(1) << (k + shift);
+      high |= u32(l + 32768);
+    }
+    u16* w = lmask + (at >> 4);
+    w[0] |= u16(m);
+    if (m >> 16) {
+      w[1] |= u16(m >> 16);
+      w[2] |= u16(m >> 32);
+      w[3] |= u16(m >> 48);
+    }
+    if (high >> 16)
+      for (int j = 0; j < tc; ++j) {
+        const int l = lv[nzp[j0 + dj * j]];
+        if (l != i16(l) && nwide < kMaxWide) {
+          wide[nwide] = l;
+          wide_at[nwide++] = u16(at + n0 + j);
+        }
+      }
+  }
+};
+bool coef_levels_enabled();
+void set_coef_levels(bool on);
+void levels_to_blocks(MbResidual& res, bool i16x16, int qp, int qpc, int qpc2);
 void dequantize_mb(const MbLevels& lv, bool i16x16, int qp, int qpc, MbResidual& out);
 void store_mb(Picture& pic, int mb, MbRec m, const MbState& s, const MbResidual* res, const u8* pcm,
               const WpEntry* wp = nullptr);
diff --git a/csrc/vep/avc_internal.h b/csrc/vep/avc_internal.h
--- a/csrc/vep/avc_internal.h
+++ b/csrc/vep/avc_internal.h
@@ -63,8 +63,6 @@
   std::unique_ptr<Impl> p_;
 };
 
-inline i16 sat16(int v) { return i16(v < -32768 ? -32768 : v > 32767 ? 32767 : v); }
-
 inline void hadamard4x4(int c[16]) {
   int t[16];
   for (int i = 0; i < 4; ++i) {
diff --git a/csrc/vep/avc_mb.cpp b/csrc/vep/avc_mb.cpp
--- a/csrc/vep/avc_mb.cpp
+++ b/csrc/vep/avc_mb.cpp
@@ -14,7 +14,12 @@
 struct Dequant {
   int ls4[6][6][16];
   int ls8[2][6][64];
+  bool flat = true;
   explicit Dequant(const h264::ScalingLists& sl) {
+    for (const auto& l : sl.l4)
+      for (u8 v : l) flat &= v == 16;
+    for (const auto& l : sl.l8)
+      for (u8 v : l) flat &= v == 16;
     for (int l = 0; l < 6; ++l)
       for (int m = 0; m < 6; ++m)
         for (int k = 0; k < 16; ++k) {
@@ -38,13 +43,6 @@
     last = sl;
   }
   return *dq;
-}
-
-inline int scale4(int c, int ls, int qp) {
-  return qp >= 24 ? (c * ls) * (1 << (qp / 6 - 4)) : (c * ls + (1 << (3 - qp / 6))) >> (4 - qp / 6);
-}
-inline int scale8(int c, int ls, int qp) {
-  return qp >= 36 ? (c * ls) * (1 << (qp / 6 - 6)) : (c * ls + (1 << (5 - qp / 6))) >> (6 - qp / 6);
 }
 
 constexpr u8 kBPart[23][2] = {{0, 0}, {1, 0}, {2, 0}, {3, 0}, {1, 1}, {1, 1}, {2, 2}, {2, 2},
@@ -86,6 +84,8 @@
       qpc_tab_[1][q] = u8(chroma_qp_bd(q - qpbd_, pps_.second_chroma_qp_index_offset, qpbdc_) + qpbdc_);
     }
     fast_direct_ = !kWrite && type_ == h264::kB && sh_.direct_spatial && sps_.direct_8x8 && !weighted_;
+    levels_ok_ = !kWrite && coef_levels_enabled() && bd_ == 8 && sps_.bit_depth_chroma == 8 && cf_ == 1 &&
+                 !env.field && dq.flat;
   }
 
   Bits* br = nullptr;
@@ -900,6 +900,11 @@
     const int q6 = qp / 6, qm = qp % 6;
     int lv[64];
     u8 nzp[64];
+    const bool lev = levels_ok_ && !(s.t8x8 && !kCabac);
+    if (lev) {
+      res.levels = true;
+      std::memset(res.lmask, 0, sizeof res.lmask);
+    }
     if (s.kind == kI16x16) {
       const int inc = kCabac ? cbf_dc_inc(mb, 0, true) : 0;
       const int nc = kCabac ? 0 : nb_.nc_luma(mb, 0);
@@ -918,18 +923,30 @@
         const int r = blk_to_raster(idx);
         i16* d = res.blk[r];
         bool nz = dcy[r] != 0;
-        std::memset(d, 0, 16 * sizeof(i16));
-        d[0] = sat16(dcy[r]);
+        if (lev) {
+          if (nz) {
+            res.lvl[16 * r] = sat16(dcy[r]);
+            res.lmask[r] = 1;
+          }
+        } else {
+          std::memset(d, 0, 16 * sizeof(i16));
+          d[0] = sat16(dcy[r]);
+        }
         if (cbp_luma) {
           const int binc = kCabac ? cbf_luma_inc(mb, r, true) : 0;
           const int bnc = kCabac ? 0 : nb_.nc_luma(mb, r);
           const int tc = read_block(kCatLumaAc, binc, bnc, 15, lv, nzp, kWrite ? want->ac[r] : nullptr);
-          for (int j = 0; j < tc; ++j) {
-            const int k = nzp[j];
-            const int pos = scan4_[k + 1];
-            const int v = scale4(lv[k], dq_.ls4[ly][qm][pos], qp);
-            d[pos] = sat16(v);
-            nz |= v != 0;
+          if (lev) {
+            res.put_levels(16 * r, nz ? 1 : 0, lv, nzp, tc, 1, !kCabac);
+            nz |= tc != 0;
+          } else {
+            for (int j = 0; j < tc; ++j) {
+              const int k = nzp[j];
+              const int pos = scan4_[k + 1];
+              const int v = scale4(lv[k], dq_.ls4[ly][qm][pos], qp);
+              d[pos] = sat16(v);
+              nz |= v != 0;
+            }
           }
           s.tc[r] = u8(tc);
           if (tc) s.cbf |= u16(1u << r);
@@ -942,7 +959,7 @@
       for (int b8 = 0; b8 < 4; ++b8) {
         if (!((cbp_luma >> b8) & 1)) continue;
         i16* d = res.b8[b8];
-        std::memset(d, 0, 64 * sizeof(i16));
+        if (!lev) std::memset(d, 0, 64 * sizeof(i16));
         bool nz = false;
         int total = 0;
         auto put = [&](int k, int level) {
@@ -953,7 +970,12 @@
         };
         if constexpr (kCabac) {
           total = read_block(kCatLuma8x8, -1, 0, 64, lv, nzp, kWrite ? want->l8[b8] : nullptr);
-          for (int j = 0; j < total; ++j) put(nzp[j], lv[nzp[j]]);
+          if (lev) {
+            res.put_levels(64 * b8, 0, lv, nzp, total, 0, false);
+            nz = total != 0;
+          } else {
+            for (int j = 0; j < total; ++j) put(nzp[j], lv[nzp[j]]);
+          }
           for (u16 w = b8_blocks(b8); w; w &= w - 1) s.tc[__builtin_ctz(w)] = u8(std::min(total, 16));
         } else {
           for (int i4 = 0; i4 < 4; ++i4) {
@@ -983,6 +1005,11 @@
         s.tc[r] = u8(tc);
         if (!tc) continue;
         s.cbf |= u16(1u << r);
+        if (lev) {
+          res.put_levels(16 * r, 0, lv, nzp, tc, 0, !kCabac);
+          res.luma |= u16(1u << r);
+          continue;
+        }
         i16* d = res.blk[r];
         std::memset(d, 0, 16 * sizeof(i16));
         bool nz = false;
@@ -1025,20 +1052,32 @@
         for (int b = 0; b < nbc; ++b) {
           i16* d = res.blk[16 + c * nbc + b];
           bool nz = dcv[c][b] != 0;
-          std::memset(d, 0, 16 * sizeof(i16));
-          d[0] = sat16(dcv[c][b]);
+          if (lev) {
+            if (nz) {
+              res.lvl[256 + 16 * (c * 4 + b)] = sat16(dcv[c][b]);
+              res.lmask[16 + c * 4 + b] = 1;
+            }
+          } else {
+            std::memset(d, 0, 16 * sizeof(i16));
+            d[0] = sat16(dcv[c][b]);
+          }
           if (cbp_chroma & 2) {
             const int binc = kCabac ? cbf_cac_inc(mb, c, b, intra) : 0;
             const int bnc = kCabac ? 0 : nb_.nc_chroma(mb, c, b, nbc);
             const int tc = read_block(kCatChromaAc, binc, bnc, 15, lv, nzp, kWrite ? want->cac[c][b] : nullptr);
             s.tcc[c][b] = u8(tc);
             if (tc) s.cbf_cac[c] |= u8(1u << b);
-            for (int j = 0; j < tc; ++j) {
-              const int k = nzp[j];
-              const int pos = scan4_[k + 1];
-              const int v = scale4(lv[k], dq_.ls4[lc][qpc[c] % 6][pos], qpc[c]);
-              d[pos] = sat16(v);
-              nz |= v != 0;
+            if (lev) {
+              res.put_levels(256 + 16 * (c * 4 + b), nz ? 1 : 0, lv, nzp, tc, 1, !kCabac);
+              nz |= tc != 0;
+            } else {
+              for (int j = 0; j < tc; ++j) {
+                const int k = nzp[j];
+                const int pos = scan4_[k + 1];
+                const int v = scale4(lv[k], dq_.ls4[lc][qpc[c] % 6][pos], qpc[c]);
+                d[pos] = sat16(v);
+                nz |= v != 0;
+              }
             }
           }
           if (nz) res.chroma |= u16(1u << (c * nbc + b));
@@ -1046,6 +1085,7 @@
       }
     }
     if constexpr (!kCabac && !kWrite) VEP_CHECK(!br->overrun(), "slice data overrun");
+    if (lev && res.nwide) levels_to_blocks(res, s.kind == kI16x16, qp, qpc_tab_[0][qp], qpc_tab_[1][qp]);
   }
 
   void emit(int mb, const MbState& s, const MbResidual& res, int i16_mode, int chroma_mode, const u8* pcm) {
@@ -1142,6 +1182,7 @@
   u8 slot_[2][33];
   u8 qpc_tab_[2][96];
   bool fast_direct_ = false;
+  bool levels_ok_ = false;
   const ColMotion* dcol_ = nullptr;
   bool dcol_long_ = false;
 };
diff --git a/csrc/vep/avc_recon.h b/csrc/vep/avc_recon.h
--- a/csrc/vep/avc_recon.h
+++ b/csrc/vep/avc_recon.h
@@ -28,6 +28,7 @@
 constexpr u8 kMbWp = 4;
 constexpr u8 kMbMv8x8 = 8;
 constexpr u8 kMbMv16 = 16;
+constexpr u8 kMbLevels = 32;
 
 struct MbRec {
   u8 kind;
@@ -111,16 +112,6 @@
   for (int k = j; k > 0; --k) w &= w - 1;
   return 16 * __builtin_ctz(w);
 }
-inline void expand_coefs(const i16* pool, const MbRec& m, i16* dense) {
-  for (int i = 0; i < kDenseCoefs; ++i) dense[i] = 0;
-  const int nw = coef_words(m);
-  const i16* v = pool + m.coef + nw;
-  for (int j = 0; j < nw; ++j) {
-    const u32 mask = u16(pool[m.coef + j]);
-    i16* d = dense + coef_word_base(m, j);
-    for (u32 b = mask; b; b &= b - 1) d[__builtin_ctz(b)] = *v++;
-  }
-}
 inline u32 coef_values(const i16* pool, const MbRec& m) {
   u32 n = 0;
   for (int j = 0, nw = coef_words(m); j < nw; ++j) n += u32(__builtin_popcount(u32(u16(pool[m.coef + j]))));
@@ -187,11 +178,15 @@
 VEP_HD int imin(int a, int b) { return a < b ? a : b; }
 VEP_HD int imax(int a, int b) { return a > b ? a : b; }
 
-VEP_HD int dequant4x4(int c, int qp, int i, int j) {
-  const int ls = 16 * norm_adjust(qp % 6, i, j);
-  if (qp >= 24) return c * ls * (1 << (qp / 6 - 4));
-  return (c * ls + (1 << (3 - qp / 6))) >> (4 - qp / 6);
-}
+VEP_HD int scale4(int c, int ls, int qp) {
+  return qp >= 24 ? (c * ls) * (1 << (qp / 6 - 4)) : (c * ls + (1 << (3 - qp / 6))) >> (4 - qp / 6);
+}
+VEP_HD int scale8(int c, int ls, int qp) {
+  return qp >= 36 ? (c * ls) * (1 << (qp / 6 - 6)) : (c * ls + (1 << (5 - qp / 6))) >> (6 - qp / 6);
+}
+VEP_HD i16 sat16(int v) { return i16(v < -32768 ? -32768 : v > 32767 ? 32767 : v); }
+
+VEP_HD int dequant4x4(int c, int qp, int i, int j) { return scale4(c, 16 * norm_adjust(qp % 6, i, j), qp); }
 
 VEP_HD void idct4x4(const i16* d, int* r) {
   int f[16];
@@ -247,6 +242,51 @@
   else if (((i & 3) == 0 && (j & 3) == 2) || ((i & 3) == 2 && (j & 3) == 0)) cls = 4;
   else cls = 5;
   return kNormAdjust8[m][cls];
+}
+
+VEP_HD i16 dequant_level4(int level, int qp, int pos) {
+  return sat16(scale4(level, 16 * norm_adjust(qp % 6, pos >> 2, pos & 3), qp));
+}
+VEP_HD i16 dequant_level8(int level, int qp, int pos) {
+  return sat16(scale8(level, 16 * norm_adjust8(qp % 6, pos >> 3, pos & 7), qp));
+}
+struct LevelWord {
+  int blk;
+  int scan0;
+  int qp;
+  bool t8;
+  bool dc;
+};
+VEP_HD LevelWord level_word(const MbRec& m, int base) {
+  static_assert(offsetof(MbRec, qp) == 1 && offsetof(MbRec, qpc) == 2 && offsetof(MbRec, qpc2) == 3, "MbRec QPs");
+  const bool chroma = base >= 256;
+  const int qp = byte_at(&m.kind, chroma ? (base >= 256 + 64 ? 3 : 2) : 1);
+  const bool t8 = !chroma && (m.flags & kMbT8x8);
+  return {t8 ? base & ~63 : base, t8 ? base & 63 : 0, qp, t8, chroma || m.kind == kI16x16};
+}
+VEP_HD void place_level(i16* dense, const LevelWord& w, int i, i16 v) {
+  if (w.t8) {
+    const int pos = kZigzag8x8[w.scan0 + i];
+    dense[w.blk + pos] = dequant_level8(v, w.qp, pos);
+  } else {
+    const int pos = kZigzag4x4[i];
+    dense[w.blk + pos] = w.dc && i == 0 ? v : dequant_level4(v, w.qp, pos);
+  }
+}
+inline void expand_coefs(const i16* pool, const MbRec& m, i16* dense) {
+  for (int i = 0; i < kDenseCoefs; ++i) dense[i] = 0;
+  const int nw = coef_words(m);
+  const i16* v = pool + m.coef + nw;
+  for (int j = 0; j < nw; ++j) {
+    const u32 mask = u16(pool[m.coef + j]);
+    i16* d = dense + coef_word_base(m, j);
+    if (m.flags & kMbLevels) {
+      const LevelWord w = level_word(m, int(d - dense));
+      for (u32 b = mask; b; b &= b - 1) place_level(dense, w, __builtin_ctz(b), *v++);
+    } else {
+      for (u32 b = mask; b; b &= b - 1) d[__builtin_ctz(b)] = *v++;
+    }
+  }
 }
 
 VEP_HD void idct8_1d(int* x) {
diff --git a/csrc/vep/gpu_avc.hip b/csrc/vep/gpu_avc.hip
--- a/csrc/vep/gpu_avc.hip
+++ b/csrc/vep/gpu_avc.hip
@@ -63,7 +63,12 @@
   wave_sync();
   if (lane < nw) {
     const VEP_DEV i16* v = pool + nw + (incl - cnt);
-    for (u32 b = mask; b; b &= b - 1) D[base + __ffs(int(b)) - 1] = *v++;
+    if (m.flags & avc::kMbLevels) {
+      const avc::LevelWord w = avc::level_word(m, base);
+      for (u32 b = mask; b; b &= b - 1) avc::place_level(D, w, __ffs(int(b)) - 1, *v++);
+    } else {
+      for (u32 b = mask; b; b &= b - 1) D[base + __ffs(int(b)) - 1] = *v++;
+    }
   }
   wave_sync();
 }
```

After: 8291. -1.8%, worse.
